# faustomorales/keras-ocr

Hardware: AMD Instinct MI355X
Metric: images/sec end-to-end Pipeline.recognize() @768x768 (higher is better)
Workload: dtype f32 (fp32 operands as 2 fp16 pieces [F(4,3) / head layers] or 3 bf16 pieces [1x1, dilated], 3 / 6 MFMA products, fp32 accumulate; fp32-class error vs fp64: tests/test_conv_gpu.py)

## Files before the change

### keras_ocr_amd/csrc/conv_w43h.hip

```cpp
#include "w43_common.h"
#include "probe_clock.h"

namespace {

#define W4H_SCALED_CONSTANTS(sc)                                                                       \
  const float k_s = (sc), k_sA = (sc) * W4_A, k_sB = (sc) * W4_B, k_sA2 = (sc) * W4_A2, k_sB2 = (sc) * W4_B2, \
              k_sA2B2 = (sc) * W4_A2B2, k_sA2PB2 = (sc) * W4_A2PB2
template <class T>
__device__ __forceinline__ T w4h_transform(const T (&d)[6], int xi, float k_s, float k_sA, float k_sB, float k_sA2, float k_sB2,
                                           float k_sA2B2, float k_sA2PB2) {
  switch (xi) {
    case 0: return (k_sA2B2 * d[0] - k_sA2PB2 * d[2]) + k_s * d[4];
    case 1: return (k_s * d[4] - k_sB2 * d[2]) + k_sA * (d[3] - W4_B2 * d[1]);
    case 2: return (k_s * d[4] - k_sB2 * d[2]) - k_sA * (d[3] - W4_B2 * d[1]);
    case 3: return (k_s * d[4] - k_sA2 * d[2]) + k_sB * (d[3] - W4_A2 * d[1]);
    case 4: return (k_s * d[4] - k_sA2 * d[2]) - k_sB * (d[3] - W4_A2 * d[1]);
    default: return (k_sA2B2 * d[1] - k_sA2PB2 * d[3]) + k_s * d[5];
  }
}

constexpr int W4H_TOP = 12;

}

template <int POOL, int GEO, int NP, int DBG = 0, int MODE = 0>
__global__ __launch_bounds__(256) void conv_w43vh_kernel(W4Params p) {
  static_assert(GEO == 1 || GEO == 2, "4 x 64 or 8 x 32 tiles");
  static_assert(!(POOL && GEO == 2), "no fused pooling on 8 x 32 tiles");
  static_assert(NP == 1 || NP == 2, "one or two fp16 pieces");
  static_assert(MODE == 0 || MODE == 1 || MODE == 2, "exact tiling, ragged, cells");
  constexpr int PR = NP == 2 ? 3 : 1;
  constexpr int NROWS = GEO == 2 ? 10 : 6;
  constexpr int QPR = GEO == 2 ? 8 : 16;
  constexpr int KHS = QPR * 8;
  constexpr int ROW_STRIDE = 2 * KHS;
  constexpr int PLANE_R = NROWS * 2 * KHS;
  constexpr int BUF_R = 6 * NP * PLANE_R;
  constexpr int TCOLS = QPR * 4;
  extern __shared__ __attribute__((aligned(16))) unsigned short As[];
  float* coef = reinterpret_cast<float*>(As + 2 * BUF_R);
  const int tid = threadIdx.x, lane = tid & 63;
  const int wn = __builtin_amdgcn_readfirstlane(tid >> 6);
  const int l31 = lane & 31, l5 = lane >> 5;
  const int nblk_n = p.Cout_pad >> 7;
  const int total = p.total_tiles;
  const int ncg = p.Cin >> 4;
  const int ns = 3 * ncg;
  const int G = gridDim.x;
  constexpr unsigned OOB = 0x80000000u;
  PROBE_T0();

  auto slot = [&](int w, int kh, int q) {
    if constexpr (GEO == 2)
      return ((w >> 1) * 2 + kh) * 128 + (w & 1) * 64 + ((q * 8) ^ (kh * 32));
    else
      return w * ROW_STRIDE + kh * KHS + ((q * 8) ^ (kh * 32));
  };
  auto tile_org = [&](int mp, int& y0, int& x0, int& nimg_o) -> long {
    if constexpr (MODE != 0) {
      const int rq = (int)w4_fdiv((unsigned)mp, p.dv_tpr), cb = mp - rq * p.tiles_per_row;
      const int nimg = (int)w4_fdiv((unsigned)rq, p.dv_rq), ro = rq - nimg * p.rq_per_img;
      y0 = (GEO == 2 ? 8 : 4) * ro;
      x0 = TCOLS * cb;
      nimg_o = nimg;
      return ((long)nimg * p.H + y0) * p.W + x0;
    } else if constexpr (GEO == 2) {
      const int rq = (int)w4_fdiv((unsigned)mp, p.dv_tpr), cb = mp - rq * p.tiles_per_row;
      const int ho = p.H >> 3;
      const int nimg = (int)w4_fdiv((unsigned)rq, p.dv_hh), ro = rq - nimg * ho;
      y0 = 8 * ro;
      x0 = 32 * cb;
      return ((long)nimg * p.H + y0) * p.W + x0;
    } else {
      const int rq = (int)w4_fdiv((unsigned)mp, p.dv_tpr), cb = mp - rq * p.tiles_per_row;
      return w4_mtile_pm0<1>(p, 2 * rq * p.tiles_per_row + cb, y0, x0);
    }
  };

  const int q4 = tid & 3, qd0 = (tid >> 2) & (QPR - 1), r0 = GEO == 2 ? (tid >> 5) : (tid >> 6);
  const int cp = tid & 7;
  const int qd1 = GEO == 2 ? ((tid >> 3) & 7) : ((tid >> 3) & 15);
  const int r1 = GEO == 2 ? 8 + ((tid >> 6) & 1) : 4 + (tid >> 7);
  int ldst[2];
  ldst[0] = slot(r0, q4 >> 1, qd0) + (q4 & 1) * 4;
  ldst[1] = slot(r1, cp >> 2, qd1) + (cp & 3) * 2;
  struct Geo {
    unsigned off0[2];
    unsigned ok;
    int e;
    int e1, qb;
    const float* base;
  };
  auto make_geo = [&](int L, Geo& g, bool& left, bool& right) __attribute__((always_inline)) {
    int mp, nt_unused;
    w4_decode(p, kocr_xcd_remap(L < total ? L : 0, total), nblk_n, mp, nt_unused);
    int y0, x0, nimg = 0;
    const long pm = tile_org(mp, y0, x0, nimg);
    g.base = p.in + (pm * p.in_cs + p.in_co) - (long)(p.W + 1) * p.in_cs;
    const int tid = wn * 64 + kocr_fresh_lane();
    const int q4 = tid & 3, qd0 = (tid >> 2) & (QPR - 1), r0 = GEO == 2 ? (tid >> 5) : (tid >> 6);
    const int cp = tid & 7;
    const int qd1 = GEO == 2 ? ((tid >> 3) & 7) : ((tid >> 3) & 15);
    const int r1 = GEO == 2 ? 8 + ((tid >> 6) & 1) : 4 + (tid >> 7);
    g.off0[0] = (unsigned)(((r0 * p.W + 4 * qd0) * p.in_cs + q4 * 4) * 4);
    g.off0[1] = (unsigned)(((r1 * p.W + 4 * qd1) * p.in_cs + cp * 2) * 4);
    g.ok = ((L < total && (unsigned)(y0 - 1 + r0) < (unsigned)p.H) ? 1u : 0u) |
           ((L < total && (unsigned)(y0 - 1 + r1) < (unsigned)p.H) ? 2u : 0u);
    g.e1 = 0;
    g.qb = QPR;
    if constexpr (MODE == 2) {
      const int j0 = (int)w4_fdiv((unsigned)x0, p.dv_wc);
      const int j1 = j0 + 1 < p.cells_per_row ? j0 + 1 : j0;
      const int c0 = __builtin_amdgcn_readfirstlane(nimg * p.cells_per_row + j0), c1 = __builtin_amdgcn_readfirstlane(nimg * p.cells_per_row + j1);
      g.e = kocr_scale_exp_bits(kocr_sload(p.amax_in + c0), W4H_TOP);
      g.e1 = kocr_scale_exp_bits(kocr_sload(p.amax_in + c1), W4H_TOP);
      const int qb = ((j0 + 1) * p.cellW - x0) >> 2;
      g.qb = qb < QPR ? qb : QPR;
    } else if constexpr (MODE == 1) {
      g.e = kocr_scale_exp_bits(kocr_sload(p.amax_in + __builtin_amdgcn_readfirstlane(nimg)), W4H_TOP);
    } else {
      g.e = kocr_scale_exp_bits(kocr_sload(p.amax_in + __builtin_amdgcn_readfirstlane((int)w4_fdiv((unsigned)pm, p.dv_hw))), W4H_TOP);
    }
    if constexpr (MODE == 1) {
      const int c0 = x0 - 1 + 4 * qd0, c1 = x0 - 1 + 4 * qd1;
      unsigned cm = 0;
#pragma unroll
      for (int k = 0; k < 6; ++k)
        cm |= ((unsigned)(c0 + k) < (unsigned)p.W ? 0u : (4u << k)) | ((unsigned)(c1 + k) < (unsigned)p.W ? 0u : (256u << k));
      g.ok |= cm;
      left = right = false;
    } else {
      left = x0 == 0;
      right = x0 + TCOLS >= p.W;
    }
  };
  Geo gc, gn;
  bool lc, rc, ln, rn;
  int ld_cg = 0;
  bool ld_next = false;
  auto load_item0 = [&](v4f (&raw)[6]) __attribute__((always_inline)) {
    if constexpr (DBG & 16) return;
    const int soff = ld_cg * 64;
    const unsigned okb = ld_next ? gn.ok : gc.ok;
    const bool ok = okb & 1u;
    const unsigned off0 = (ld_next ? gn.off0[0] : gc.off0[0]) | (ok ? 0u : OOB);
    const bool left = (ld_next ? ln : lc) && qd0 == 0, right = (ld_next ? rn : rc) && qd0 == QPR - 1;
    const unsigned stride = (unsigned)(p.in_cs * 4);
    const __amdgpu_buffer_rsrc_t rsrc = w4_rsrc(ld_next ? gn.base : gc.base, 0x80000000u);
#pragma unroll
    for (int k = 0; k < 6; ++k) {
      const unsigned padk = MODE == 1 ? ((okb << (29 - k)) & OOB)
                                      : ((k == 0 ? (left ? OOB : 0u) : 0u) | (k == 5 ? (right ? OOB : 0u) : 0u));
      if constexpr (DBG & 128)
        raw[k] = __builtin_bit_cast(v4f, __builtin_amdgcn_raw_buffer_load_b128(w4_rsrc(p.in, 0x80000000u), (unsigned)((tid & 63) * 16 + (tid >> 6) * 8192 + k * 1024), soff & 0xFFF, 0));
      else if constexpr (DBG & 64)
        raw[k] = __builtin_bit_cast(v4f, __builtin_amdgcn_raw_buffer_load_b128(w4_rsrc(p.in, 0x80000000u), ((off0 + k * stride) | padk) & 0x8003FFF0u, soff & 0xFFF, 0));
      else
      raw[k] = __builtin_bit_cast(v4f, __builtin_amdgcn_raw_buffer_load_b128(rsrc, (off0 + k * stride) | padk, soff, 0));
    }
  };
  auto load_item1 = [&](v2f (&raw)[6]) __attribute__((always_inline)) {
    if constexpr (DBG & 16) return;
    const int soff = ld_cg * 64;
    const unsigned okb = ld_next ? gn.ok : gc.ok;
    const bool ok = (okb >> 1) & 1u;
    const unsigned off0 = (ld_next ? gn.off0[1] : gc.off0[1]) | (ok ? 0u : OOB);
    const bool left = (ld_next ? ln : lc) && qd1 == 0, right = (ld_next ? rn : rc) && qd1 == QPR - 1;
    const unsigned stride = (unsigned)(p.in_cs * 4);
    const __amdgpu_buffer_rsrc_t rsrc = w4_rsrc(ld_next ? gn.base : gc.base, 0x80000000u);
#pragma unroll
    for (int k = 0; k < 6; ++k) {
      const unsigned padk = MODE == 1 ? ((okb << (23 - k)) & OOB)
                                      : ((k == 0 ? (left ? OOB : 0u) : 0u) | (k == 5 ? (right ? OOB : 0u) : 0u));
      if constexpr (DBG & 128)
        raw[k] = __builtin_bit_cast(v2f, __builtin_amdgcn_raw_buffer_load_b64(w4_rsrc(p.in, 0x80000000u), (unsigned)((tid & 63) * 8 + (tid >> 6) * 8192 + 6144 + k * 512), soff & 0xFFF, 0));
      else if constexpr (DBG & 64)
        raw[k] = __builtin_bit_cast(v2f, __builtin_amdgcn_raw_buffer_load_b64(w4_rsrc(p.in, 0x80000000u), ((off0 + k * stride) | padk) & 0x8003FFF8u, soff & 0xFFF, 0));
      else
      raw[k] = __builtin_bit_cast(v2f, __builtin_amdgcn_raw_buffer_load_b64(rsrc, (off0 + k * stride) | padk, soff, 0));
    }
  };
  auto advance = [&]() __attribute__((always_inline)) {
    const bool wrap = ld_cg == ncg - 1;
    ld_cg = wrap ? 0 : ld_cg + 1;
    ld_next = ld_next || wrap;
  };
  auto produce4 = [&](const v4f (&d)[6], unsigned short* bufp, int xi, int it, float sc0, float sc1, int scq) __attribute__((always_inline)) {
    const float sk = MODE == 2 ? (qd0 < scq ? sc0 : sc1) : sc0;
    unsigned short* dst = bufp + xi * NP * PLANE_R + ldst[it];
    if constexpr (DBG & 1) {
      const u2v r = __builtin_bit_cast(u2v, __builtin_shufflevector(d[xi], d[xi], 0, 1));
      *reinterpret_cast<u2v*>(dst) = r;
      if constexpr (NP == 2) *reinterpret_cast<u2v*>(dst + PLANE_R) = r;
      return;
    }
    v4f V;
    if constexpr (MODE == 2) {
      V = w4_transform(d, xi) * sk;
    } else {
      W4H_SCALED_CONSTANTS(sk);
      V = w4h_transform(d, xi, k_s, k_sA, k_sB, k_sA2, k_sB2, k_sA2B2, k_sA2PB2);
    }
    if constexpr (NP == 2) {
      u2v h, l;
      kocr_split4_h(V, h, l);
      *reinterpret_cast<u2v*>(dst) = h;
      *reinterpret_cast<u2v*>(dst + PLANE_R) = l;
    } else {
      *reinterpret_cast<u2v*>(dst) = u2v{__builtin_bit_cast(unsigned, hf2{(_Float16)V[0], (_Float16)V[1]}),
                                         __builtin_bit_cast(unsigned, hf2{(_Float16)V[2], (_Float16)V[3]})};
    }
  };
  auto produce2 = [&](const v2f (&d)[6], unsigned short* bufp, int xi, float sc0, float sc1, int scq) __attribute__((always_inline)) {
    const float sk = MODE == 2 ? (qd1 < scq ? sc0 : sc1) : sc0;
    unsigned short* dst = bufp + xi * NP * PLANE_R + ldst[1];
    if constexpr (DBG & 1) {
      const unsigned r = __float_as_uint(d[xi][0]);
      *reinterpret_cast<unsigned*>(dst) = r;
      if constexpr (NP == 2) *reinterpret_cast<unsigned*>(dst + PLANE_R) = r;
      return;
    }
    v2f V;
    if constexpr (MODE == 2) {
      V = w4_transform(d, xi) * sk;
    } else {
      W4H_SCALED_CONSTANTS(sk);
      V = w4h_transform(d, xi, k_s, k_sA, k_sB, k_sA2, k_sB2, k_sA2B2, k_sA2PB2);
    }
    if constexpr (NP == 2) {
      unsigned h, l;
      kocr_split2_h(V, h, l);
      *reinterpret_cast<unsigned*>(dst) = h;
      *reinterpret_cast<unsigned*>(dst + PLANE_R) = l;
    } else {
      *reinterpret_cast<unsigned*>(dst) = __builtin_bit_cast(unsigned, hf2{(_Float16)V[0], (_Float16)V[1]});
    }
  };
  v4f raw0[6];
  v2f raw1[6];

  const int ntiles32 = p.Cout_pad >> 5;
  const unsigned w_step = (unsigned)ntiles32 * 12 * 64 * 16;
  const __amdgpu_buffer_rsrc_t wrsrc = w4_rsrc(reinterpret_cast<const float*>(p.wgt), 0x7FFFFFFFu);
  const unsigned wlane = (unsigned)lane * 16u;
  auto w_tile = [&](int nt) { return (unsigned)__builtin_amdgcn_readfirstlane((nt * 4 + wn) * 12 * 64 * 16); };
  hf8 bw[2][6][NP];
  f16v acc[6][2];
  const int a_lane = GEO == 2 ? slot(l31 >> 3, l5, l31 & 7) : slot(l31 >> 4, l5, l31 & 15);
  const int a_lane1 = GEO == 2 ? slot((l31 >> 3) + 1, l5, l31 & 7) : 0;
  auto load_a = [&](hf8 (&a)[2][NP], const unsigned short* bufp, int ky, int xi) __attribute__((always_inline)) {
    if constexpr (DBG & 8) return;
    const unsigned short* plane = bufp + xi * NP * PLANE_R;
#pragma unroll
    for (int s = NP - 1; s >= 0; --s)
#pragma unroll
      for (int m = 0; m < 2; ++m) {
        int off;
        if constexpr (GEO == 2) {
          const int c = ky + 4 * m;
          off = ((c & 1) ? a_lane1 : a_lane) + (c >> 1) * 256;
        } else {
          off = a_lane + (ky + 2 * m) * ROW_STRIDE;
        }
        a[m][s] = *reinterpret_cast<const hf8*>(plane + s * PLANE_R + off);
      }
  };
  auto mfma_pt = [&](const hf8 (&a)[2][NP], const hf8 (&b)[NP], int xi) __attribute__((always_inline)) {
    if constexpr (DBG & 4) {
#pragma unroll
      for (int m = 0; m < 2; ++m)
#pragma unroll
        for (int s = 0; s < NP; ++s) acc[xi][m][s] += __builtin_bit_cast(v4f, a[m][s])[0] + __builtin_bit_cast(v4f, b[s])[0];
      return;
    }
    if constexpr (NP == 2) {
#pragma unroll
      for (int m = 0; m < 2; ++m) acc[xi][m] = __builtin_amdgcn_mfma_f32_32x32x16_f16(a[m][1], b[0], acc[xi][m], 0, 0, 0);
#pragma unroll
      for (int m = 0; m < 2; ++m) acc[xi][m] = __builtin_amdgcn_mfma_f32_32x32x16_f16(a[m][0], b[1], acc[xi][m], 0, 0, 0);
    }
#pragma unroll
    for (int m = 0; m < 2; ++m) acc[xi][m] = __builtin_amdgcn_mfma_f32_32x32x16_f16(a[m][0], b[0], acc[xi][m], 0, 0, 0);
  };
  hf8 a0[2][NP], a1[2][NP];
  auto step = [&](auto ky_c, auto slot_c, const unsigned short* bufc, unsigned short* bufn, unsigned w_next, float sc0, float sc1, int scq) __attribute__((always_inline)) {
    constexpr int KY = decltype(ky_c)::value;
    constexpr int SLOT = decltype(slot_c)::value;
    auto load_b = [&](int xi) __attribute__((always_inline)) {
      if constexpr (DBG & 2) return;
#pragma unroll
      for (int s = 0; s < NP; ++s)
        bw[SLOT][xi][s] = __builtin_bit_cast(hf8, __builtin_amdgcn_raw_buffer_load_b128(wrsrc, wlane, (int)(w_next + (unsigned)(xi * 2 + s) * 1024u), 0));
    };
    auto produce = [&](int xi) __attribute__((always_inline)) {
      if constexpr (KY == 0) produce4(raw0, bufn, xi, 0, sc0, sc1, scq);
      if constexpr (KY == 1) produce2(raw1, bufn, xi, sc0, sc1, scq);
    };
    auto interleave = [&]() __attribute__((always_inline)) {
      __builtin_amdgcn_sched_group_barrier(0x100, 2 * NP, 0);
      if constexpr (KY < 2) {
        constexpr int VPG = (KY == 0 ? 30 : 16) / (2 * PR - 1) + 1;
#pragma unroll
        for (int i = 0; i < 2 * PR - 1; ++i) {
          __builtin_amdgcn_sched_group_barrier(0x008, 1, 0);
          __builtin_amdgcn_sched_group_barrier(0x002, VPG, 0);
        }
        __builtin_amdgcn_sched_group_barrier(0x200, NP, 0);
        __builtin_amdgcn_sched_group_barrier(0x008, 1, 0);
      } else {
        __builtin_amdgcn_sched_group_barrier(0x008, 2 * PR, 0);
      }
    };
#pragma unroll
    for (int q = 0; q < 3; ++q) {
      __builtin_amdgcn_sched_barrier(0);
      load_a(a1, bufc, KY, 2 * q + 1);
      produce(2 * q);
      mfma_pt(a0, bw[SLOT][2 * q], 2 * q);
      interleave();
      __builtin_amdgcn_sched_barrier(0);
      load_b(2 * q);
      __builtin_amdgcn_sched_barrier(0);
      if (q < 2) {
        load_a(a0, bufc, KY, 2 * q + 2);
        produce(2 * q + 1);
        mfma_pt(a1, bw[SLOT][2 * q + 1], 2 * q + 1);
        interleave();
      } else if constexpr (KY < 2) {
        load_a(a0, bufc, KY + 1, 0);
        produce(5);
        mfma_pt(a1, bw[SLOT][5], 5);
        interleave();
      } else {
        if constexpr (!(DBG & 32)) __syncthreads();
        load_a(a0, bufn, 0, 0);
        __builtin_amdgcn_sched_barrier(0);
        mfma_pt(a1, bw[SLOT][5], 5);
      }
      __builtin_amdgcn_sched_barrier(0);
      load_b(2 * q + 1);
    }
  };

  w4_stage_coef(p, coef, tid);
  make_geo(blockIdx.x, gc, lc, rc);
  make_geo(blockIdx.x + G, gn, ln, rn);
  load_item0(raw0);
  load_item1(raw1);
  advance();
  {
    int mp0, nt0;
    w4_decode(p, kocr_xcd_remap(blockIdx.x, total), nblk_n, mp0, nt0);
    const unsigned w0 = w_tile(nt0);
#pragma unroll
    for (int st = 0; st < 2; ++st)
#pragma unroll
      for (int xi = 0; xi < 6; ++xi)
#pragma unroll
        for (int s = 0; s < NP; ++s)
          bw[st][xi][s] = __builtin_bit_cast(hf8, __builtin_amdgcn_raw_buffer_load_b128(wrsrc, wlane, (int)(w0 + st * w_step + (unsigned)(xi * 2 + s) * 1024u), 0));
  }
#pragma unroll
  for (int xi = 0; xi < 6; ++xi) {
    produce4(raw0, As, xi, 0, kocr_pow2(gc.e), kocr_pow2(gc.e1), gc.qb);
    produce2(raw1, As, xi, kocr_pow2(gc.e), kocr_pow2(gc.e1), gc.qb);
  }
  load_item0(raw0);
  load_item1(raw1);
  advance();
  __syncthreads();
  load_a(a0, As, 0, 0);

  PROBE_RESTART();
  for (int L = blockIdx.x; L < total; L += G) {
    int mp, nt, mp_n, nt_n;
    w4_decode(p, kocr_xcd_remap(L, total), nblk_n, mp, nt);
    w4_decode(p, kocr_xcd_remap(L + G < total ? L + G : L, total), nblk_n, mp_n, nt_n);
    const unsigned w_ptr = w_tile(nt), w_after = w_tile(nt_n);
    auto w_at = [&](int s) { return s < ns ? w_ptr + (unsigned)s * w_step : w_after + (unsigned)(s - ns) * w_step; };
    const float s_cur = kocr_pow2(gc.e), s_nxt = kocr_pow2(gn.e);
    const float s_cur1 = kocr_pow2(gc.e1), s_nxt1 = kocr_pow2(gn.e1);
    const int qb_nxt = gn.qb;
    const float unscale = kocr_pow2(-gc.e);
    const float unscale1 = kocr_pow2(-gc.e1);
    const int qb_cur = gc.qb;
#pragma unroll
    for (int x = 0; x < 6; ++x)
#pragma unroll
      for (int m = 0; m < 2; ++m)
#pragma unroll
        for (int r = 0; r < 16; ++r) acc[x][m][r] = 0.f;
    PROBE_T(5);
    __builtin_amdgcn_s_waitcnt(0x0F70);
    PROBE_T(4);
    for (int cg = 0; cg < ncg; cg += 2) {
      using I0 = std::integral_constant<int, 0>;
      using I1 = std::integral_constant<int, 1>;
      using I2 = std::integral_constant<int, 2>;
      step(I0{}, I0{}, As, As + BUF_R, w_at(3 * cg + 2), s_cur, s_cur1, qb_cur);
      load_item0(raw0);
      step(I1{}, I1{}, As, As + BUF_R, w_at(3 * cg + 3), s_cur, s_cur1, qb_cur);
      load_item1(raw1);
      advance();
      step(I2{}, I0{}, As, As + BUF_R, w_at(3 * cg + 4), s_cur, s_cur1, qb_cur);
      const bool same = cg + 2 < ncg;
      const float s_odd = same ? s_cur : s_nxt, s_odd1 = same ? s_cur1 : s_nxt1;
      const int qb_odd = same ? qb_cur : qb_nxt;
      step(I0{}, I1{}, As + BUF_R, As, w_at(3 * cg + 5), s_odd, s_odd1, qb_odd);
      load_item0(raw0);
      step(I1{}, I0{}, As + BUF_R, As, w_at(3 * cg + 6), s_odd, s_odd1, qb_odd);
      load_item1(raw1);
      advance();
      step(I2{}, I1{}, As + BUF_R, As, w_at(3 * cg + 7), s_odd, s_odd1, qb_odd);
    }
    PROBE_T(0);

    {
      const int lane_e = kocr_fresh_lane();
      const int l31e = lane_e & 31, l5e = lane_e >> 5;
      const int n = (nt * 4 + wn) * 32 + l31e;
      int ty0, tx0, timg = 0;
      const long tpm = tile_org(mp, ty0, tx0, timg);
      int nimg, nimg1 = 0, cell0_x = 0;
      if constexpr (MODE == 2) {
        const int j0 = (int)w4_fdiv((unsigned)tx0, p.dv_wc);
        const int j1 = j0 + 1 < p.cells_per_row ? j0 + 1 : j0;
        nimg = __builtin_amdgcn_readfirstlane(timg * p.cells_per_row + j0);
        nimg1 = __builtin_amdgcn_readfirstlane(timg * p.cells_per_row + j1);
        cell0_x = j0 * p.cellW;
      } else if constexpr (MODE == 1) {
        nimg = __builtin_amdgcn_readfirstlane(timg);
      } else {
        nimg = __builtin_amdgcn_readfirstlane((int)w4_fdiv((unsigned)tpm, p.dv_hw));
      }
      const unsigned seen_out = p.amax_out ? kocr_amax_peek(p.amax_out + nimg) : 0u;
      const unsigned seen_pool = p.amax_pool ? kocr_amax_peek(p.amax_pool + nimg) : 0u;
      unsigned seen_out1 = 0u, seen_pool1 = 0u;
      if constexpr (MODE == 2) {
        seen_out1 = p.amax_out ? kocr_amax_peek(p.amax_out + nimg1) : 0u;
        seen_pool1 = p.amax_pool ? kocr_amax_peek(p.amax_pool + nimg1) : 0u;
      }
      const float pa = coef[n] * unscale, pb = coef[p.Cout_pad + n];
      const float pa1 = coef[n] * unscale1;
      const bool has_post = p.post_a != nullptr;
      const float qa = coef[2 * p.Cout_pad + n], qb = coef[3 * p.Cout_pad + n];
      const bool live = n < p.Cout;
      const float lo = p.relu ? 0.f : -INFINITY;
      auto act = [&](float v, float a) { return fmaxf(v * a + pb, lo); };
      const int l5q = 4 * l5e;
      auto qx_of = [&](int r) { return GEO == 2 ? (r & 3) + l5q : (r & 3) + 8 * ((r >> 2) & 1) + l5q; };
      auto first_row = [&](int m, int r) { return m == 0 && (GEO == 2 ? (r >> 2) == 0 : r < 8); };
#pragma unroll
      for (int m = 0; m < 2; ++m)
#pragma unroll
        for (int r = 0; r < 16; ++r) {
          float par = pa;
          if constexpr (MODE == 2) par = qx_of(r) < qb_cur ? pa : pa1;
          const float m0 = acc[0][m][r], m1 = acc[1][m][r], m2 = acc[2][m][r], m3 = acc[3][m][r], m4 = acc[4][m][r],
                      m5 = acc[5][m][r];
          const float s12 = m1 + m2, d12 = m1 - m2, s34 = m3 + m4, d34 = m3 - m4;
          acc[0][m][r] = act((m0 + s12) + s34, par);
          acc[1][m][r] = act(W4_A * d12 + W4_B * d34, par);
          acc[2][m][r] = act(W4_A2 * s12 + W4_B2 * s34, par);
          acc[3][m][r] = act((W4_A3 * d12 + W4_B3 * d34) + m5, par);
        }
      if (has_post) {
#pragma unroll
        for (int j = 0; j < 4; ++j)
#pragma unroll
          for (int m = 0; m < 2; ++m)
#pragma unroll
            for (int r = 0; r < 16; ++r) acc[j][m][r] = acc[j][m][r] * qa + qb;
      }
      if constexpr (MODE == 2) {
        const bool top = ty0 == 0;
#pragma unroll
        for (int r = 0; r < 16; ++r) {
          const int qx = qx_of(r);
          const int cx = tx0 + 4 * qx - (qx < qb_cur ? cell0_x : cell0_x + p.cellW);
#pragma unroll
          for (int j = 0; j < 4; ++j) {
            const bool v = cx + j < p.cellWv;
#pragma unroll
            for (int m = 0; m < 2; ++m) acc[j][m][r] = (v && !(top && first_row(m, r))) ? acc[j][m][r] : 0.f;
          }
        }
      }
      int ocs4 = p.out_cs * 4;
      asm volatile("" : "+s"(ocs4));
      int pcs4 = p.pool_cs * 4;
      asm volatile("" : "+s"(pcs4));
      if (p.amax_out || p.amax_pool) {
        if constexpr (MODE == 2) {
          float mx0 = 0.f, mx1 = 0.f;
#pragma unroll
          for (int r = 0; r < 16; ++r) {
            float mq = 0.f;
#pragma unroll
            for (int j = 0; j < 4; ++j)
#pragma unroll
              for (int m = 0; m < 2; ++m) mq = fmaxf(mq, fabsf(acc[j][m][r]));
            const bool first = qx_of(r) < qb_cur;
            mx0 = fmaxf(mx0, first ? mq : 0.f);
            mx1 = fmaxf(mx1, first ? 0.f : mq);
          }
          mx0 = live ? mx0 : 0.f;
          mx1 = live ? mx1 : 0.f;
          if (p.amax_out) kocr_amax_update_known(p.amax_out + nimg, mx0, seen_out);
          if (p.amax_pool) kocr_amax_update_known(p.amax_pool + nimg, mx0, seen_pool);
          if (qb_cur < QPR) {
            if (p.amax_out) kocr_amax_update_known(p.amax_out + nimg1, mx1, seen_out1);
            if (p.amax_pool) kocr_amax_update_known(p.amax_pool + nimg1, mx1, seen_pool1);
          }
        } else {
          float mx = 0.f;
#pragma unroll
          for (int j = 0; j < 4; ++j)
#pragma unroll
            for (int m = 0; m < 2; ++m)
#pragma unroll
              for (int r = 0; r < 16; ++r) mx = fmaxf(mx, fabsf(acc[j][m][r]));
          mx = live ? mx : 0.f;
          if (p.amax_out) kocr_amax_update_known(p.amax_out + nimg, mx, seen_out);
          if (p.amax_pool) kocr_amax_update_known(p.amax_pool + nimg, mx, seen_pool);
        }
      }
      PROBE_T(2);
      if constexpr (GEO == 2) {
        const __amdgpu_buffer_rsrc_t ro = w4_rsrc(p.out + (tpm * p.out_cs + p.out_co), 0x7FFFFFFFu);
        const unsigned vo = live ? (unsigned)((16 * l5e * p.out_cs + n) * 4) : OOB;
        const int wlim = p.W - tx0 - 16 * l5e;
#pragma unroll
        for (int m = 0; m < 2; ++m)
#pragma unroll
          for (int r = 0; r < 16; ++r) {
            const int px = (4 * m + (r >> 2)) * p.W + 4 * (r & 3);
            if (MODE == 1 && ty0 + 4 * m + (r >> 2) >= p.H) continue;
#pragma unroll
            for (int j = 0; j < 4; ++j) {
              const unsigned vom = MODE == 1 ? (4 * (r & 3) + j < wlim ? vo : OOB) : vo;
              __builtin_amdgcn_raw_buffer_store_b32(__float_as_uint(acc[j][m][r]), ro, vom, (px + j) * ocs4, 0);
            }
          }
      } else {
#pragma unroll
        for (int m = 0; m < 2; ++m) {
          const long pm = tpm + (long)2 * m * p.W;
          const int x0 = tx0;
          if (!POOL || p.write_full) {
            const __amdgpu_buffer_rsrc_t ro = w4_rsrc(p.out + (pm * p.out_cs + p.out_co), 0x7FFFFFFFu);
            const unsigned vo = live ? (unsigned)((16 * l5e * p.out_cs + n) * 4) : OOB;
            if constexpr (MODE == 1) {
              const int wlim = p.W - tx0 - 16 * l5e;
#pragma unroll
              for (int h = 0; h < 2; ++h) {
                if (ty0 + 2 * m + h >= p.H) continue;
#pragma unroll
                for (int r = 0; r < 8; ++r) {
                  const int px = 4 * ((r & 3) + 8 * (r >> 2));
#pragma unroll
                  for (int j = 0; j < 4; ++j)
                    __builtin_amdgcn_raw_buffer_store_b32(__float_as_uint(acc[j][m][r + 8 * h]), ro, px + j < wlim ? vo : OOB,
                                                          (px + j + h * p.W) * ocs4, 0);
                }
              }
            } else {
#pragma unroll
              for (int r = 0; r < 8; ++r) {
                const int px = 4 * ((r & 3) + 8 * (r >> 2));
#pragma unroll
                for (int j = 0; j < 4; ++j) {
                  __builtin_amdgcn_raw_buffer_store_b32(__float_as_uint(acc[j][m][r]), ro, vo, (px + j) * ocs4, 0);
                  __builtin_amdgcn_raw_buffer_store_b32(__float_as_uint(acc[j][m][r + 8]), ro, vo, (px + j + p.W) * ocs4, 0);
                }
              }
            }
          }
          if constexpr (POOL) {
            long pp0;
            if constexpr (MODE == 1)
              pp0 = ((long)timg * (p.H >> 1) + (ty0 >> 1) + m) * (p.W >> 1) + (x0 >> 1);
            else
              pp0 = ((pm - x0) >> 2) + (x0 >> 1);
            const __amdgpu_buffer_rsrc_t rp = w4_rsrc(p.pool_out + (pp0 * p.pool_cs + p.pool_co), 0x7FFFFFFFu);
            const unsigned vp = live ? (unsigned)((8 * l5e * p.pool_cs + n) * 4) : OOB;
            if (MODE == 1 && (ty0 >> 1) + m >= (p.H >> 1)) continue;
            const int plim = (p.W >> 1) - (x0 >> 1) - 8 * l5e;
            const bool ztop = MODE == 2 && ty0 == 0 && m == 0;
#pragma unroll
            for (int r = 0; r < 8; ++r) {
              const int pq = 2 * ((r & 3) + 8 * (r >> 2));
              float v0 = fmaxf(fmaxf(acc[0][m][r], acc[1][m][r]), fmaxf(acc[0][m][r + 8], acc[1][m][r + 8]));
              float v1 = fmaxf(fmaxf(acc[2][m][r], acc[3][m][r]), fmaxf(acc[2][m][r + 8], acc[3][m][r + 8]));
              if constexpr (MODE == 2) {
                v0 = ztop ? 0.f : v0;
                v1 = ztop ? 0.f : v1;
              }
              __builtin_amdgcn_raw_buffer_store_b32(__float_as_uint(v0), rp, (MODE != 1 || pq < plim) ? vp : OOB, pq * pcs4, 0);
              __builtin_amdgcn_raw_buffer_store_b32(__float_as_uint(v1), rp, (MODE != 1 || pq + 1 < plim) ? vp : OOB, (pq + 1) * pcs4, 0);
            }
          }
        }
      }
      PROBE_T(3);
    }
    gc = gn;
    lc = ln;
    rc = rn;
    make_geo(L + 2 * G, gn, ln, rn);
    ld_next = false;
    PROBE_T(1);
  }
  PROBE_TEND(tid == 0, 0, 6);
}

template <int POOL, int NP, int MODE = 0, int OCC = 1>
__global__ __launch_bounds__(256, OCC) void conv_w43rh_kernel(W4Params p) {
  static_assert(MODE == 0 || MODE == 1, "exact tiling or ragged");
  constexpr int NBW = 3;
  constexpr int PR = NP == 2 ? 3 : 1;
  constexpr int NROWS = 6, QPR = 16, KHS = QPR * 8, ROW_STRIDE = 2 * KHS, PLANE_R = NROWS * ROW_STRIDE;
  constexpr int BUF_R = 6 * NP * PLANE_R;
  constexpr int TCOLS = QPR * 4;
  extern __shared__ __attribute__((aligned(16))) unsigned short As[];
  float* coef = reinterpret_cast<float*>(OCC == 2 ? As + 2 * BUF_R : As + BUF_R + 4 * 16 * 64 * 8);
  const int tid = threadIdx.x, lane = tid & 63;
  const int wave = __builtin_amdgcn_readfirstlane(tid >> 6);
  const int wn = wave & 1, ph = wave >> 1;
  const int l31 = lane & 31, l5 = lane >> 5;
  const int total = p.total_tiles;
  const int ncg = p.Cin >> 4;
  const int G = gridDim.x;
  constexpr unsigned OOB = 0x80000000u;

  auto tile_mt = [&](int mp, int m) {
    const int rq = (int)w4_fdiv((unsigned)mp, p.dv_tpr), cb = mp - rq * p.tiles_per_row;
    return (2 * rq + m) * p.tiles_per_row + cb;
  };
  auto mtile_org = [&](int mp, int m, int& y0, int& x0, int& nimg_o) -> long {
    if constexpr (MODE == 1) {
      const int rq = (int)w4_fdiv((unsigned)mp, p.dv_tpr), cb = mp - rq * p.tiles_per_row;
      const int nimg = (int)w4_fdiv((unsigned)rq, p.dv_rq), ro = rq - nimg * p.rq_per_img;
      y0 = 4 * ro + 2 * m;
      x0 = TCOLS * cb;
      nimg_o = nimg;
      return ((long)nimg * p.H + y0) * p.W + x0;
    } else {
      const long pm = w4_mtile_pm0<1>(p, tile_mt(mp, m), y0, x0);
      nimg_o = (int)w4_fdiv((unsigned)pm, p.dv_hw);
      return pm;
    }
  };

  const int q4 = tid & 3, qd0 = (tid >> 2) & (QPR - 1), r0 = tid >> 6;
  const int cp = tid & 7, qd1 = (tid >> 3) & 15, r1 = 4 + (tid >> 7);
  int ldst[2];
  ldst[0] = r0 * ROW_STRIDE + (q4 >> 1) * KHS + (((qd0 * 8) ^ ((q4 >> 1) * 32)) + (q4 & 1) * 4);
  ldst[1] = r1 * ROW_STRIDE + (cp >> 2) * KHS + (((qd1 * 8) ^ ((cp >> 2) * 32)) + (cp & 3) * 2);
  struct Geo {
    unsigned off0[2];
    unsigned ok;
    int e;
    const float* base;
  };
  auto make_geo = [&](int L, Geo& g, bool& left, bool& right) __attribute__((always_inline)) {
    const int mp = kocr_xcd_remap(L < total ? L : 0, total);
    int y0, x0, nimg;
    const long pm = mtile_org(mp, 0, y0, x0, nimg);
    g.base = p.in + (pm * p.in_cs + p.in_co) - (long)(p.W + 1) * p.in_cs;
    const int tid = wave * 64 + kocr_fresh_lane();
    const int q4 = tid & 3, qd0 = (tid >> 2) & (QPR - 1), r0 = tid >> 6;
    const int cp = tid & 7, qd1 = (tid >> 3) & 15, r1 = 4 + (tid >> 7);
    g.off0[0] = (unsigned)(((r0 * p.W + 4 * qd0) * p.in_cs + q4 * 4) * 4);
    g.off0[1] = (unsigned)(((r1 * p.W + 4 * qd1) * p.in_cs + cp * 2) * 4);
    g.ok = ((L < total && (unsigned)(y0 - 1 + r0) < (unsigned)p.H) ? 1u : 0u) |
           ((L < total && (unsigned)(y0 - 1 + r1) < (unsigned)p.H) ? 2u : 0u);
    g.e = kocr_scale_exp_bits(kocr_sload(p.amax_in + __builtin_amdgcn_readfirstlane(nimg)), W4H_TOP);
    if constexpr (MODE == 1) {
      const int c0 = x0 - 1 + 4 * qd0, c1 = x0 - 1 + 4 * qd1;
      unsigned cm = 0;
#pragma unroll
      for (int k = 0; k < 6; ++k)
        cm |= ((unsigned)(c0 + k) < (unsigned)p.W ? 0u : (4u << k)) | ((unsigned)(c1 + k) < (unsigned)p.W ? 0u : (256u << k));
      g.ok |= cm;
      left = right = false;
    } else {
      left = x0 == 0;
      right = x0 + TCOLS >= p.W;
    }
  };
  Geo gc, gn;
  bool lc, rc, ln, rn;
  int ld_cg = 0;
  bool ld_next = false;
  auto load_item0 = [&](v4f (&raw)[6]) __attribute__((always_inline)) {
    const int soff = ld_cg * 64;
    const unsigned okb = ld_next ? gn.ok : gc.ok;
    const bool ok = okb & 1u;
    const unsigned off0 = (ld_next ? gn.off0[0] : gc.off0[0]) | (ok ? 0u : OOB);
    const bool left = (ld_next ? ln : lc) && qd0 == 0, right = (ld_next ? rn : rc) && qd0 == QPR - 1;
    const unsigned stride = (unsigned)(p.in_cs * 4);
    const __amdgpu_buffer_rsrc_t rsrc = w4_rsrc(ld_next ? gn.base : gc.base, 0x80000000u);
#pragma unroll
    for (int k = 0; k < 6; ++k) {
      const unsigned padk = MODE == 1 ? ((okb << (29 - k)) & OOB) : ((k == 0 ? (left ? OOB : 0u) : 0u) | (k == 5 ? (right ? OOB : 0u) : 0u));
      raw[k] = __builtin_bit_cast(v4f, __builtin_amdgcn_raw_buffer_load_b128(rsrc, (off0 + k * stride) | padk, soff, 0));
    }
  };
  auto load_item1 = [&](v2f (&raw)[6]) __attribute__((always_inline)) {
    const int soff = ld_cg * 64;
    const unsigned okb = ld_next ? gn.ok : gc.ok;
    const bool ok = (okb >> 1) & 1u;
    const unsigned off0 = (ld_next ? gn.off0[1] : gc.off0[1]) | (ok ? 0u : OOB);
    const bool left = (ld_next ? ln : lc) && qd1 == 0, right = (ld_next ? rn : rc) && qd1 == QPR - 1;
    const unsigned stride = (unsigned)(p.in_cs * 4);
    const __amdgpu_buffer_rsrc_t rsrc = w4_rsrc(ld_next ? gn.base : gc.base, 0x80000000u);
#pragma unroll
    for (int k = 0; k < 6; ++k) {
      const unsigned padk = MODE == 1 ? ((okb << (23 - k)) & OOB) : ((k == 0 ? (left ? OOB : 0u) : 0u) | (k == 5 ? (right ? OOB : 0u) : 0u));
      raw[k] = __builtin_bit_cast(v2f, __builtin_amdgcn_raw_buffer_load_b64(rsrc, (off0 + k * stride) | padk, soff, 0));
    }
  };
  auto advance = [&]() __attribute__((always_inline)) {
    const bool wrap = ld_cg == ncg - 1;
    ld_cg = wrap ? 0 : ld_cg + 1;
    ld_next = ld_next || wrap;
  };
  auto produce4 = [&](const v4f (&d)[6], unsigned short* bufp, int xi, float sk) __attribute__((always_inline)) {
    W4H_SCALED_CONSTANTS(sk);
    const v4f V = w4h_transform(d, xi, k_s, k_sA, k_sB, k_sA2, k_sB2, k_sA2B2, k_sA2PB2);
    unsigned short* dst = bufp + xi * NP * PLANE_R + ldst[0];
    if constexpr (NP == 2) {
      u2v h, l;
      kocr_split4_h(V, h, l);
      *reinterpret_cast<u2v*>(dst) = h;
      *reinterpret_cast<u2v*>(dst + PLANE_R) = l;
    } else {
      *reinterpret_cast<u2v*>(dst) = u2v{__builtin_bit_cast(unsigned, hf2{(_Float16)V[0], (_Float16)V[1]}),
                                         __builtin_bit_cast(unsigned, hf2{(_Float16)V[2], (_Float16)V[3]})};
    }
  };
  auto produce2 = [&](const v2f (&d)[6], unsigned short* bufp, int xi, float sk) __attribute__((always_inline)) {
    W4H_SCALED_CONSTANTS(sk);
    const v2f V = w4h_transform(d, xi, k_s, k_sA, k_sB, k_sA2, k_sB2, k_sA2B2, k_sA2PB2);
    unsigned short* dst = bufp + xi * NP * PLANE_R + ldst[1];
    if constexpr (NP == 2) {
      unsigned h, l;
      kocr_split2_h(V, h, l);
      *reinterpret_cast<unsigned*>(dst) = h;
      *reinterpret_cast<unsigned*>(dst + PLANE_R) = l;
    } else {
      *reinterpret_cast<unsigned*>(dst) = __builtin_bit_cast(unsigned, hf2{(_Float16)V[0], (_Float16)V[1]});
    }
  };
  v4f raw0[1][6];
  v2f raw1[1][6];

  constexpr unsigned w_step = 2u * 12 * 64 * 16;
  const __amdgpu_buffer_rsrc_t wrsrc = w4_rsrc(reinterpret_cast<const float*>(p.wgt), 0x7FFFFFFFu);
  const unsigned wlane = (unsigned)lane * 16u;
  const unsigned w_wave = (unsigned)__builtin_amdgcn_readfirstlane(wn * 12 * 64 * 16 + 3 * ph * 2 * 64 * 16);
  const int ns = 3 * ncg;
  hf8 bw[NBW][NP];
  f16v acc[3][2];
  const int a_lane = (l31 >> 4) * ROW_STRIDE + l5 * KHS + (((l31 & 15) * 8) ^ (l5 * 32));
  constexpr int M_OFF = 2 * ROW_STRIDE;
  auto load_a = [&](hf8 (&a)[2][NP], const unsigned short* bufp, int ky, int pl) __attribute__((always_inline)) {
    const unsigned short* base = bufp + a_lane + ky * ROW_STRIDE + (3 * ph + pl) * NP * PLANE_R;
#pragma unroll
    for (int s = NP - 1; s >= 0; --s)
#pragma unroll
      for (int m = 0; m < 2; ++m) a[m][s] = *reinterpret_cast<const hf8*>(base + s * PLANE_R + m * M_OFF);
  };
  auto mfma_grp = [&](const hf8 (&a)[2][NP], int pl, int bi) __attribute__((always_inline)) {
    if constexpr (NP == 2) {
#pragma unroll
      for (int m = 0; m < 2; ++m) acc[pl][m] = __builtin_amdgcn_mfma_f32_32x32x16_f16(a[m][1], bw[bi][0], acc[pl][m], 0, 0, 0);
#pragma unroll
      for (int m = 0; m < 2; ++m) acc[pl][m] = __builtin_amdgcn_mfma_f32_32x32x16_f16(a[m][0], bw[bi][1], acc[pl][m], 0, 0, 0);
    }
#pragma unroll
    for (int m = 0; m < 2; ++m) acc[pl][m] = __builtin_amdgcn_mfma_f32_32x32x16_f16(a[m][0], bw[bi][0], acc[pl][m], 0, 0, 0);
  };
  hf8 a0[2][NP], a1[2][NP];
  auto phase = [&](const unsigned short* bufc, unsigned short* bufn, int s0, int flip, float sk) __attribute__((always_inline)) {
    v4f(&r0)[6] = raw0[0];
    v2f(&r1)[6] = raw1[0];
#pragma unroll
    for (int g = 0; g < 9; ++g) {
      __builtin_amdgcn_sched_barrier(0);
      const int ky = g / 3, pp = g - ky * 3;
      hf8(&cur)[2][NP] = ((g & 1) ^ flip) ? a1 : a0;
      hf8(&nxt)[2][NP] = ((g & 1) ^ flip) ? a0 : a1;
      const int nchunks = (g % 3 == 0) ? 2 : 1;
      const int c0 = (g / 3) * 4 + (g % 3 == 0 ? 0 : g % 3 + 1);
      if (g < 8) load_a(nxt, bufc, (g + 1) / 3, (g + 1) % 3);
#pragma unroll
      for (int c = c0; c < c0 + nchunks; ++c) {
        if (c < 6)
          produce4(r0, bufn, c, sk);
        else
          produce2(r1, bufn, c - 6, sk);
      }
      if (g < 8) {
        mfma_grp(cur, pp, pp);
        __builtin_amdgcn_sched_group_barrier(0x100, 2 * NP, 0);
        auto ilv = [&](auto v_c, auto st_c) __attribute__((always_inline)) {
          constexpr int V = decltype(v_c)::value, ST = decltype(st_c)::value;
#pragma unroll
          for (int i = 0; i < 2 * PR - 1; ++i) {
            __builtin_amdgcn_sched_group_barrier(0x008, 1, 0);
            __builtin_amdgcn_sched_group_barrier(0x002, V, 0);
          }
          __builtin_amdgcn_sched_group_barrier(0x200, ST, 0);
        };
        const bool half = c0 >= 6;
        if (nchunks == 2) {
          if (half)
            ilv(std::integral_constant<int, PR == 3 ? 3 : 20>{}, std::integral_constant<int, 2 * NP>{});
          else
            ilv(std::integral_constant<int, PR == 3 ? 5 : 44>{}, std::integral_constant<int, 2 * NP>{});
        } else {
          if (half)
            ilv(std::integral_constant<int, PR == 3 ? 2 : 10>{}, std::integral_constant<int, NP>{});
          else
            ilv(std::integral_constant<int, PR == 3 ? 2 : 22>{}, std::integral_constant<int, NP>{});
        }
        __builtin_amdgcn_sched_group_barrier(0x008, 1, 0);
      } else {
        __syncthreads();
        load_a(nxt, bufn, 0, 0);
        __builtin_amdgcn_sched_barrier(0);
        mfma_grp(cur, pp, pp);
      }
      __builtin_amdgcn_sched_barrier(0);
      {
        int sn = s0 + ky + 1;
        sn = sn >= ns ? sn - ns : sn;
        const unsigned wq = w_wave + (unsigned)sn * w_step;
#pragma unroll
        for (int s = 0; s < NP; ++s)
          bw[pp][s] = __builtin_bit_cast(hf8, __builtin_amdgcn_raw_buffer_load_b128(wrsrc, wlane, (int)(wq + (unsigned)(pp * 2 + s) * 1024u), 0));
      }
      if (g == 3) load_item0(r0);
    }
    load_item1(r1);
    advance();
  };

  w4_stage_coef(p, coef, tid);
  make_geo(blockIdx.x, gc, lc, rc);
  make_geo(blockIdx.x + G, gn, ln, rn);
  load_item0(raw0[0]);
  load_item1(raw1[0]);
  advance();
#pragma unroll
  for (int g = 0; g < NBW; ++g)
#pragma unroll
    for (int s = 0; s < NP; ++s)
      bw[g][s] = __builtin_bit_cast(hf8, __builtin_amdgcn_raw_buffer_load_b128(wrsrc, wlane, (int)(w_wave + (unsigned)(g / 3) * w_step + (unsigned)((g % 3) * 2 + s) * 1024u), 0));
#pragma unroll
  for (int xi = 0; xi < 6; ++xi) {
    produce4(raw0[0], As, xi, kocr_pow2(gc.e));
    produce2(raw1[0], As, xi, kocr_pow2(gc.e));
  }
  load_item0(raw0[0]);
  load_item1(raw1[0]);
  advance();
  __syncthreads();
  load_a(a0, As, 0, 0);

  PROBE_T0();
  for (int L = blockIdx.x; L < total; L += G) {
    const int mp = kocr_xcd_remap(L, total);
    const float s_cur = kocr_pow2(gc.e), s_nxt = kocr_pow2(gn.e);
    const float unscale = kocr_pow2(-gc.e);
#pragma unroll
    for (int x = 0; x < 3; ++x)
#pragma unroll
      for (int m = 0; m < 2; ++m)
#pragma unroll
        for (int r = 0; r < 16; ++r) acc[x][m][r] = 0.f;
    PROBE_T(5);
    __builtin_amdgcn_s_waitcnt(0x0F70);
    PROBE_T(4);
    for (int cg = 0; cg < ncg; cg += 2) {
      phase(As, As + BUF_R, 3 * cg, 0, s_cur);
      phase(As + BUF_R, As, 3 * cg + 3, 1, cg + 2 < ncg ? s_cur : s_nxt);
    }

    PROBE_T(0);
    {
      const int lane_e = kocr_fresh_lane();
      const int l31e = lane_e & 31, l5e = lane_e >> 5;
      const int n = wn * 32 + l31e;
      int y0, x0, timg;
      const long pm = mtile_org(mp, ph, y0, x0, timg);
      const int nimg = __builtin_amdgcn_readfirstlane(timg);
      const unsigned seen_out = p.amax_out ? kocr_amax_peek(p.amax_out + nimg) : 0u;
      const unsigned seen_pool = p.amax_pool ? kocr_amax_peek(p.amax_pool + nimg) : 0u;
      const float pa = coef[n] * unscale, pb = coef[p.Cout_pad + n];
      const bool has_post = p.post_a != nullptr;
      const float qa = coef[2 * p.Cout_pad + n], qb = coef[3 * p.Cout_pad + n];
      const bool live = n < p.Cout;
      const float lo = p.relu ? 0.f : -INFINITY;
      auto act = [&](float v) { return fmaxf(v * pa + pb, lo); };
      v4f* xch = reinterpret_cast<v4f*>(As + BUF_R);
      float out[4][16];
      auto halves = [&](auto ph_c) __attribute__((always_inline)) {
        constexpr int PH = decltype(ph_c)::value;
        auto partial = [&](auto m_c, int r, float (&o)[4]) __attribute__((always_inline)) {
          constexpr int M = decltype(m_c)::value;
          const float u = acc[0][M][r], v = acc[1][M][r], w = acc[2][M][r];
          if constexpr (PH == 0) {
            const float s12 = v + w, d12 = v - w;
            o[0] = u + s12;
            o[1] = W4_A * d12;
            o[2] = W4_A2 * s12;
            o[3] = W4_A3 * d12;
          } else {
            const float s34 = u + v, d34 = u - v;
            o[0] = s34;
            o[1] = W4_B * d34;
            o[2] = W4_B2 * s34;
            o[3] = W4_B3 * d34 + w;
          }
        };
        if constexpr (OCC == 1) {
#pragma unroll
          for (int r = 0; r < 16; ++r) {
            float o[4];
            partial(std::integral_constant<int, 1 - PH>{}, r, o);
            xch[(wave * 16 + r) * 64 + lane_e] = v4f{o[0], o[1], o[2], o[3]};
          }
        }
#pragma unroll
        for (int r = 0; r < 16; ++r) {
          float o[4];
          partial(std::integral_constant<int, PH>{}, r, o);
#pragma unroll
          for (int j = 0; j < 4; ++j) out[j][r] = o[j];
        }
        if constexpr (OCC == 2) {
#pragma unroll
          for (int h = 0; h < 2; ++h) {
#pragma unroll
            for (int r = 8 * h; r < 8 * h + 8; ++r) {
              float o[4];
              partial(std::integral_constant<int, 1 - PH>{}, r, o);
              xch[(wave * 8 + r - 8 * h) * 64 + lane_e] = v4f{o[0], o[1], o[2], o[3]};
            }
            __syncthreads();
#pragma unroll
            for (int r = 8 * h; r < 8 * h + 8; ++r) {
              const v4f q = xch[((wave ^ 2) * 8 + r - 8 * h) * 64 + lane_e];
#pragma unroll
              for (int j = 0; j < 4; ++j) out[j][r] += q[j];
            }
            __syncthreads();
          }
        }
      };
      if (ph == 0)
        halves(std::integral_constant<int, 0>{});
      else
        halves(std::integral_constant<int, 1>{});
      if constexpr (OCC == 1) {
        __syncthreads();
#pragma unroll
        for (int r = 0; r < 16; ++r) {
          const v4f q = xch[((wave ^ 2) * 16 + r) * 64 + lane_e];
#pragma unroll
          for (int j = 0; j < 4; ++j) out[j][r] = act(out[j][r] + q[j]);
        }
      } else {
#pragma unroll
        for (int r = 0; r < 16; ++r)
#pragma unroll
          for (int j = 0; j < 4; ++j) out[j][r] = act(out[j][r]);
      }
      if (has_post) {
#pragma unroll
        for (int r = 0; r < 16; ++r)
#pragma unroll
          for (int j = 0; j < 4; ++j) out[j][r] = out[j][r] * qa + qb;
      }
      if constexpr (OCC == 1) __syncthreads();
      int ocs4 = p.out_cs * 4;
      asm volatile("" : "+s"(ocs4));
      int pcs4 = p.pool_cs * 4;
      asm volatile("" : "+s"(pcs4));
      if (p.amax_out || p.amax_pool) {
        float mx = 0.f;
#pragma unroll
        for (int j = 0; j < 4; ++j)
#pragma unroll
          for (int r = 0; r < 16; ++r) mx = fmaxf(mx, fabsf(out[j][r]));
        mx = live ? mx : 0.f;
        if (p.amax_out) kocr_amax_update_known(p.amax_out + nimg, mx, seen_out);
        if (p.amax_pool) kocr_amax_update_known(p.amax_pool + nimg, mx, seen_pool);
      }
      PROBE_T(2);
      if (!POOL || p.write_full) {
        const __amdgpu_buffer_rsrc_t ro = w4_rsrc(p.out + (pm * p.out_cs + p.out_co), 0x7FFFFFFFu);
        const unsigned vo = live ? (unsigned)((16 * l5e * p.out_cs + n) * 4) : OOB;
        if constexpr (MODE == 1) {
          const int wlim = p.W - x0 - 16 * l5e;
#pragma unroll
          for (int h = 0; h < 2; ++h) {
            if (y0 + h >= p.H) continue;
#pragma unroll
            for (int r = 0; r < 8; ++r) {
              const int px = 4 * ((r & 3) + 8 * (r >> 2));
#pragma unroll
              for (int j = 0; j < 4; ++j)
                __builtin_amdgcn_raw_buffer_store_b32(__float_as_uint(out[j][r + 8 * h]), ro, px + j < wlim ? vo : OOB, (px + j + h * p.W) * ocs4, 0);
            }
          }
        } else {
#pragma unroll
          for (int r = 0; r < 8; ++r) {
            const int px = 4 * ((r & 3) + 8 * (r >> 2));
#pragma unroll
            for (int j = 0; j < 4; ++j) {
              __builtin_amdgcn_raw_buffer_store_b32(__float_as_uint(out[j][r]), ro, vo, (px + j) * ocs4, 0);
              __builtin_amdgcn_raw_buffer_store_b32(__float_as_uint(out[j][r + 8]), ro, vo, (px + j + p.W) * ocs4, 0);
            }
          }
        }
      }
      if constexpr (POOL) {
        long pp0;
        if constexpr (MODE == 1)
          pp0 = ((long)timg * (p.H >> 1) + (y0 >> 1)) * (p.W >> 1) + (x0 >> 1);
        else
          pp0 = ((pm - x0) >> 2) + (x0 >> 1);
        const __amdgpu_buffer_rsrc_t rp = w4_rsrc(p.pool_out + (pp0 * p.pool_cs + p.pool_co), 0x7FFFFFFFu);
        const unsigned vp = live ? (unsigned)((8 * l5e * p.pool_cs + n) * 4) : OOB;
        const bool prow = MODE != 1 || (y0 >> 1) < (p.H >> 1);
        const int plim = (p.W >> 1) - (x0 >> 1) - 8 * l5e;
        if (prow) {
#pragma unroll
          for (int r = 0; r < 8; ++r) {
            const int pq = 2 * ((r & 3) + 8 * (r >> 2));
            const float v0 = fmaxf(fmaxf(out[0][r], out[1][r]), fmaxf(out[0][r + 8], out[1][r + 8]));
            const float v1 = fmaxf(fmaxf(out[2][r], out[3][r]), fmaxf(out[2][r + 8], out[3][r + 8]));
            __builtin_amdgcn_raw_buffer_store_b32(__float_as_uint(v0), rp, (MODE != 1 || pq < plim) ? vp : OOB, pq * pcs4, 0);
            __builtin_amdgcn_raw_buffer_store_b32(__float_as_uint(v1), rp, (MODE != 1 || pq + 1 < plim) ? vp : OOB, (pq + 1) * pcs4, 0);
          }
        }
      }
      PROBE_T(3);
    }
    gc = gn;
    lc = ln;
    rc = rn;
    make_geo(L + 2 * G, gn, ln, rn);
    ld_next = false;
    PROBE_T(1);
  }
  PROBE_TEND(tid == 0, 0, 6);
}

template <int NP, int DIL = 0>
__global__ __launch_bounds__(256) void conv_w43fh_kernel(W4Params p) {
  constexpr int PR = NP == 2 ? 3 : 1;
  constexpr int PLANE_F = PLANE;
  constexpr int BUF_F = 6 * NP * PLANE_F;
  extern __shared__ __attribute__((aligned(16))) unsigned short As[];
  float* coef = reinterpret_cast<float*>(As + 2 * BUF_F);
  const int tid = threadIdx.x, lane = tid & 63;
  const int wn = __builtin_amdgcn_readfirstlane(tid >> 6);
  const int l31 = lane & 31, l5 = lane >> 5;
  const int nblk_n = p.Cout_pad >> 7;
  const int total = p.total_tiles;
  const int ns = p.nsteps;
  const int G = gridDim.x;
  const int hw = p.H * p.W;
  constexpr unsigned OOB = 0x80000000u;

  const int qi = tid >> 2, q4 = tid & 3;
  const int ldst = ((qi >> 5) * 2 + (q4 >> 1)) * KH_STRIDE + ((((qi & 31) * 8) ^ ((q4 >> 1) * 32)) + (q4 & 1) * 4);
  struct Geo {
    unsigned goff[6];
    int gy;
    bool gok;
    float s;
    int e0, e1;
    const float* base;
  };
  const int dd = DIL ? p.dil : 1;
  auto make_geo = [&](int L, Geo& g) __attribute__((always_inline)) {
    int mp, nt_unused;
    w4_decode(p, kocr_xcd_remap(L < total ? L : 0, total), nblk_n, mp, nt_unused);
    const int tid_f = wn * 64 + kocr_fresh_lane();
    const int qi = tid_f >> 2, q4 = tid_f & 3;
    if constexpr (DIL) {
      const unsigned q0 = (unsigned)mp * 64u;
      const unsigned nq = (unsigned)(p.Mtotal >> 2);
      const unsigned row_a = w4_fdiv(q0 < nq ? q0 : nq - 1, p.dv_qpr);
      g.base = p.in + ((long)row_a * p.W * p.in_cs + p.in_co) - (long)(dd * p.W + dd) * p.in_cs;
      const unsigned qg = q0 + (unsigned)qi;
      g.gok = L < total && qg < nq;
      const unsigned qc = qg < nq ? qg : nq - 1;
      const unsigned row = w4_fdiv(qc, p.dv_qpr);
      const int qr = (int)(qc - row * (unsigned)p.qpr);
      const int qd = (int)w4_fdiv((unsigned)qr, p.dv_dil);
      const int x0 = qd * 4 * dd + (qr - qd * dd);
      const unsigned nimg = w4_fdiv(row, p.dv_h);
      g.gy = (int)(row - nimg * (unsigned)p.H);
      const int n0 = __builtin_amdgcn_readfirstlane((int)w4_fdiv(row_a, p.dv_h));
      const int n1 = (n0 + 1 < p.Mtotal / (p.H * p.W)) ? n0 + 1 : n0;
      g.e0 = kocr_scale_exp_bits(kocr_sload(p.amax_in + n0), W4H_TOP);
      g.e1 = kocr_scale_exp_bits(kocr_sload(p.amax_in + n1), W4H_TOP);
      g.s = kocr_pow2((int)nimg == n0 ? g.e0 : g.e1);
      const int rel = (int)(row - row_a) * p.W + x0;
#pragma unroll
      for (int k = 0; k < 6; ++k) {
        const bool pad = (k == 0 && x0 < dd) || (k == 5 && x0 + 4 * dd >= p.W);
        g.goff[k] = pad ? OOB : (unsigned)(((rel + k * dd) * p.in_cs + q4 * 4) * 4);
      }
      return;
    }
    const long pm_a = (long)mp * 256;
    g.base = p.in + (pm_a * p.in_cs + p.in_co) - (long)(p.W + 1) * p.in_cs;
    const int rel = 4 * qi;
    const long gp = pm_a + rel;
    g.gok = L < total && gp < p.Mtotal;
    const unsigned gpc = (unsigned)(gp < p.Mtotal ? gp : (long)p.Mtotal - 1);
    const unsigned row = w4_fdiv(gpc, p.dv_w), nimg = w4_fdiv(gpc, p.dv_hw);
    const int x0 = (int)(gpc - row * (unsigned)p.W);
    g.gy = (int)(row - nimg * (unsigned)p.H);
    const unsigned pmc = (unsigned)(pm_a < (long)p.Mtotal ? pm_a : (long)p.Mtotal - 1);
    const int n0 = __builtin_amdgcn_readfirstlane((int)w4_fdiv(pmc, p.dv_hw));
    const int n1 = ((long)(n0 + 1) * hw < (long)p.Mtotal) ? n0 + 1 : n0;
    g.e0 = kocr_scale_exp_bits(kocr_sload(p.amax_in + n0), W4H_TOP);
    g.e1 = kocr_scale_exp_bits(kocr_sload(p.amax_in + n1), W4H_TOP);
    g.s = kocr_pow2((int)nimg == n0 ? g.e0 : g.e1);
#pragma unroll
    for (int k = 0; k < 6; ++k) {
      const bool pad = (k == 0 && x0 < 1) || (k == 5 && x0 + 4 >= p.W);
      g.goff[k] = pad ? OOB : (unsigned)(((rel + k) * p.in_cs + q4 * 4) * 4);
    }
  };
  Geo gc, gn;
  int ld_ky = 0, ld_cg = 0;
  bool ld_next = false;
  const int ncg = p.Cin >> 4;
  auto load_raw = [&](v4f (&raw)[6]) __attribute__((always_inline)) {
    const int soff = (ld_ky * dd * p.W * p.in_cs + ld_cg * 16) * 4;
    const int gy = ld_next ? gn.gy : gc.gy;
    const bool ok = (ld_next ? gn.gok : gc.gok) & ((unsigned)(gy + dd * (ld_ky - 1)) < (unsigned)p.H);
    const unsigned kill = ok ? 0u : OOB;
    const __amdgpu_buffer_rsrc_t rsrc = w4_rsrc(ld_next ? gn.base : gc.base, 0x80000000u);
#pragma unroll
    for (int k = 0; k < 6; ++k)
      raw[k] = __builtin_bit_cast(v4f, __builtin_amdgcn_raw_buffer_load_b128(rsrc, (ld_next ? gn.goff[k] : gc.goff[k]) | kill, soff, 0));
    const bool wrap_ky = ld_ky == 2;
    ld_ky = wrap_ky ? 0 : ld_ky + 1;
    const bool wrap_cg = wrap_ky && ld_cg == ncg - 1;
    ld_cg = wrap_cg ? 0 : (wrap_ky ? ld_cg + 1 : ld_cg);
    ld_next = ld_next || wrap_cg;
  };
  auto produce_point = [&](const v4f (&d)[6], unsigned short* bufp, int xi, float sk) __attribute__((always_inline)) {
    W4H_SCALED_CONSTANTS(sk);
    const v4f V = w4h_transform(d, xi, k_s, k_sA, k_sB, k_sA2, k_sB2, k_sA2B2, k_sA2PB2);
    unsigned short* dst = bufp + xi * NP * PLANE_F + ldst;
    if constexpr (NP == 2) {
      u2v h, l;
      kocr_split4_h(V, h, l);
      *reinterpret_cast<u2v*>(dst) = h;
      *reinterpret_cast<u2v*>(dst + PLANE_F) = l;
    } else {
      *reinterpret_cast<u2v*>(dst) = u2v{__builtin_bit_cast(unsigned, hf2{(_Float16)V[0], (_Float16)V[1]}),
                                         __builtin_bit_cast(unsigned, hf2{(_Float16)V[2], (_Float16)V[3]})};
    }
  };

  const int ntiles32 = p.Cout_pad >> 5;
  const size_t w_step = (size_t)ntiles32 * 12 * 64 * 8;
  auto w_tile = [&](int nt) { return p.wgt + ((size_t)(nt * 4 + wn) * 12 * 64 + lane) * 8; };
  hf8 bw[6][NP];
  f16v acc[6][2];
  const int a_lane = l5 * KH_STRIDE + ((l31 * 8) ^ (l5 * 32));
  auto load_a = [&](hf8 (&a)[2][NP], const unsigned short* bufp, int xi) __attribute__((always_inline)) {
    const unsigned short* base = bufp + xi * NP * PLANE_F + a_lane;
#pragma unroll
    for (int s = NP - 1; s >= 0; --s)
#pragma unroll
      for (int m = 0; m < 2; ++m) a[m][s] = *reinterpret_cast<const hf8*>(base + s * PLANE_F + m * 2 * KH_STRIDE);
  };
  auto mfma_pt = [&](const hf8 (&a)[2][NP], int xi) __attribute__((always_inline)) {
    if constexpr (NP == 2) {
#pragma unroll
      for (int m = 0; m < 2; ++m) acc[xi][m] = __builtin_amdgcn_mfma_f32_32x32x16_f16(a[m][1], bw[xi][0], acc[xi][m], 0, 0, 0);
#pragma unroll
      for (int m = 0; m < 2; ++m) acc[xi][m] = __builtin_amdgcn_mfma_f32_32x32x16_f16(a[m][0], bw[xi][1], acc[xi][m], 0, 0, 0);
    }
#pragma unroll
    for (int m = 0; m < 2; ++m) acc[xi][m] = __builtin_amdgcn_mfma_f32_32x32x16_f16(a[m][0], bw[xi][0], acc[xi][m], 0, 0, 0);
  };
  hf8 a0[2][NP], a1[2][NP];
  auto step = [&](const unsigned short* bufc, unsigned short* bufn, const v4f (&raw)[6], const unsigned short* w_next, float sk)
                  __attribute__((always_inline)) {
    auto load_b = [&](int xi) __attribute__((always_inline)) {
#pragma unroll
      for (int s = 0; s < NP; ++s) bw[xi][s] = *reinterpret_cast<const hf8*>(w_next + (size_t)(xi * 2 + s) * 64 * 8);
    };
    auto interleave = [&]() __attribute__((always_inline)) {
      __builtin_amdgcn_sched_group_barrier(0x100, 2 * NP, 0);
      constexpr int VPG = 30 / (2 * PR - 1) + 1;
#pragma unroll
      for (int i = 0; i < 2 * PR - 1; ++i) {
        __builtin_amdgcn_sched_group_barrier(0x008, 1, 0);
        __builtin_amdgcn_sched_group_barrier(0x002, VPG, 0);
      }
      __builtin_amdgcn_sched_group_barrier(0x200, NP, 0);
      __builtin_amdgcn_sched_group_barrier(0x008, 1, 0);
    };
#pragma unroll
    for (int q = 0; q < 3; ++q) {
      __builtin_amdgcn_sched_barrier(0);
      load_a(a1, bufc, 2 * q + 1);
      produce_point(raw, bufn, 2 * q, sk);
      mfma_pt(a0, 2 * q);
      interleave();
      __builtin_amdgcn_sched_barrier(0);
      load_b(2 * q);
      __builtin_amdgcn_sched_barrier(0);
      if (q < 2) {
        load_a(a0, bufc, 2 * q + 2);
        produce_point(raw, bufn, 2 * q + 1, sk);
        mfma_pt(a1, 2 * q + 1);
        interleave();
      } else {
        produce_point(raw, bufn, 5, sk);
        __syncthreads();
        load_a(a0, bufn, 0);
        __builtin_amdgcn_sched_barrier(0);
        mfma_pt(a1, 5);
      }
      __builtin_amdgcn_sched_barrier(0);
      load_b(2 * q + 1);
    }
  };

  w4_stage_coef(p, coef, tid);
  make_geo(blockIdx.x, gc);
  make_geo(blockIdx.x + G, gn);
  v4f rawA[6], rawB[6];
  load_raw(rawA);
  load_raw(rawB);
  {
    int mp0, nt0;
    w4_decode(p, kocr_xcd_remap(blockIdx.x, total), nblk_n, mp0, nt0);
    const unsigned short* w0 = w_tile(nt0);
#pragma unroll
    for (int xi = 0; xi < 6; ++xi)
#pragma unroll
      for (int s = 0; s < NP; ++s) bw[xi][s] = *reinterpret_cast<const hf8*>(w0 + (size_t)(xi * 2 + s) * 64 * 8);
  }
#pragma unroll
  for (int xi = 0; xi < 6; ++xi) produce_point(rawA, As, xi, gc.s);
  load_raw(rawA);
  __syncthreads();
  load_a(a0, As, 0);

  PROBE_T0();
  for (int L = blockIdx.x; L < total; L += G) {
    int mp, nt, mp_n, nt_n;
    w4_decode(p, kocr_xcd_remap(L, total), nblk_n, mp, nt);
    w4_decode(p, kocr_xcd_remap(L + G < total ? L + G : L, total), nblk_n, mp_n, nt_n);
    const unsigned short* w_ptr = w_tile(nt);
    const unsigned short* w_after = w_tile(nt_n);
    const float s_cur = gc.s, s_nxt = gn.s;
#pragma unroll
    for (int x = 0; x < 6; ++x)
#pragma unroll
      for (int m = 0; m < 2; ++m)
#pragma unroll
        for (int r = 0; r < 16; ++r) acc[x][m][r] = 0.f;
    __builtin_amdgcn_s_waitcnt(0x0F70);
    for (int s = 0; s < ns; s += 2) {
      step(As, As + BUF_F, rawB, w_ptr + (size_t)(s + 1) * w_step, s_cur);
      load_raw(rawB);
      step(As + BUF_F, As, rawA, s + 2 < ns ? w_ptr + (size_t)(s + 2) * w_step : w_after, s + 2 < ns ? s_cur : s_nxt);
      load_raw(rawA);
    }
    PROBE_T(0);
    const int e0c = gc.e0, e1c = gc.e1;

    {
      const int lane_e = kocr_fresh_lane();
      const int l31e = lane_e & 31, l5e = lane_e >> 5;
      const int n = (nt * 4 + wn) * 32 + l31e;
      const long pm0 = (long)mp * 256;
      const long pm0c = pm0 < (long)p.Mtotal ? pm0 : (long)p.Mtotal - 1;
      const int n0 = __builtin_amdgcn_readfirstlane((int)w4_fdiv((unsigned)pm0c, p.dv_hw));
      const long b1 = ((long)(n0 + 1) * hw - pm0) >> 2;
      const int qb = __builtin_amdgcn_readfirstlane((int)(b1 < 64 ? b1 : 64));
      const int n1 = ((long)(n0 + 1) * hw < (long)p.Mtotal) ? n0 + 1 : n0;
      unsigned seen0 = 0, seen1 = 0;
      if (p.amax_out) {
        seen0 = kocr_amax_peek(p.amax_out + n0);
        seen1 = kocr_amax_peek(p.amax_out + n1);
      }
      const float u0 = kocr_pow2(-e0c), u1 = kocr_pow2(-e1c);
      const float pre_a = coef[n], pb = coef[p.Cout_pad + n];
      const float pa0 = pre_a * u0, pa1 = pre_a * u1;
      const bool has_post = p.post_a != nullptr;
      const bool live = n < p.Cout;
      const float lo = p.relu ? 0.f : -INFINITY;
      const int qlim = (int)((((long)p.Mtotal - pm0) >> 2) < 64 ? (((long)p.Mtotal - pm0) >> 2) : 64);
      const int l5q = 4 * l5e;
#pragma unroll
      for (int m = 0; m < 2; ++m)
#pragma unroll
        for (int r = 0; r < 16; ++r) {
          const int q = m * 32 + (r & 3) + 8 * (r >> 2) + l5q;
          const float pa = q < qb ? pa0 : pa1;
          const float m0 = acc[0][m][r], m1 = acc[1][m][r], m2 = acc[2][m][r], m3 = acc[3][m][r], m4 = acc[4][m][r],
                      m5 = acc[5][m][r];
          const float s12 = m1 + m2, d12 = m1 - m2, s34 = m3 + m4, d34 = m3 - m4;
          acc[0][m][r] = fmaxf(((m0 + s12) + s34) * pa + pb, lo);
          acc[1][m][r] = fmaxf((W4_A * d12 + W4_B * d34) * pa + pb, lo);
          acc[2][m][r] = fmaxf((W4_A2 * s12 + W4_B2 * s34) * pa + pb, lo);
          acc[3][m][r] = fmaxf(((W4_A3 * d12 + W4_B3 * d34) + m5) * pa + pb, lo);
        }
      if (has_post) {
        const float qa = coef[2 * p.Cout_pad + n], qb_ = coef[3 * p.Cout_pad + n];
#pragma unroll
        for (int j = 0; j < 4; ++j)
#pragma unroll
          for (int m = 0; m < 2; ++m)
#pragma unroll
            for (int r = 0; r < 16; ++r) acc[j][m][r] = acc[j][m][r] * qa + qb_;
      }
      if (!DIL && p.Wv) {
#pragma unroll
        for (int m = 0; m < 2; ++m)
#pragma unroll
          for (int r = 0; r < 16; ++r) {
            const int q = m * 32 + (r & 3) + 8 * (r >> 2) + l5q;
            const unsigned pq = (unsigned)(pm0 + 4 * q);
            const int x0 = (int)(pq - w4_fdiv(pq, p.dv_w) * (unsigned)p.W);
#pragma unroll
            for (int j = 0; j < 4; ++j) acc[j][m][r] = x0 + j < p.Wv ? acc[j][m][r] : 0.f;
          }
      }
      if (p.amax_out) {
        float mx0 = 0.f, mx1 = 0.f;
#pragma unroll
        for (int m = 0; m < 2; ++m)
#pragma unroll
          for (int r = 0; r < 16; ++r) {
            const int q = m * 32 + (r & 3) + 8 * (r >> 2) + l5q;
            const float mq = (live && q < qlim) ? fmaxf(fmaxf(fabsf(acc[0][m][r]), fabsf(acc[1][m][r])), fmaxf(fabsf(acc[2][m][r]), fabsf(acc[3][m][r]))) : 0.f;
            mx0 = fmaxf(mx0, q < qb ? mq : 0.f);
            mx1 = fmaxf(mx1, q < qb ? 0.f : mq);
          }
        kocr_amax_update_known(p.amax_out + n0, mx0, seen0);
        if (qb < 64) kocr_amax_update_known(p.amax_out + n1, mx1, seen1);
      }
      PROBE_T(2);
      int ocs4 = p.out_cs * 4;
      asm volatile("" : "+s"(ocs4));
      if constexpr (DIL) {
        const unsigned q0 = (unsigned)mp * 64u;
        const unsigned row_a = w4_fdiv(q0, p.dv_qpr);
        const __amdgpu_buffer_rsrc_t ro = w4_rsrc(p.out + ((long)row_a * p.W * p.out_cs + p.out_co), 0x7FFFFFFFu);
        const int dstep = dd * ocs4;
#pragma unroll
        for (int m = 0; m < 2; ++m)
#pragma unroll
          for (int r = 0; r < 16; ++r) {
            const int q = m * 32 + (r & 3) + 8 * (r >> 2) + l5q;
            const unsigned qg = q0 + (unsigned)q;
            const unsigned row = w4_fdiv(qg, p.dv_qpr);
            const int qr = (int)(qg - row * (unsigned)p.qpr);
            const int qd = (int)w4_fdiv((unsigned)qr, p.dv_dil);
            const int x0 = qd * 4 * dd + (qr - qd * dd);
            const unsigned vo = (live && q < qlim) ? (unsigned)((((int)(row - row_a) * p.W + x0) * p.out_cs + n) * 4) : OOB;
#pragma unroll
            for (int j = 0; j < 4; ++j) __builtin_amdgcn_raw_buffer_store_b32(__float_as_uint(acc[j][m][r]), ro, vo, j * dstep, 0);
          }
      } else {
      const long rem = ((long)p.Mtotal - pm0) * ocs4;
      const __amdgpu_buffer_rsrc_t ro =
          w4_rsrc(p.out + (pm0 * p.out_cs + p.out_co), rem < 0x7FFFFFFFL ? (unsigned)(rem > 0 ? rem : 0) : 0x7FFFFFFFu);
      const unsigned vo = live ? (unsigned)((16 * l5e * p.out_cs + n) * 4) : OOB;
#pragma unroll
      for (int m = 0; m < 2; ++m)
#pragma unroll
        for (int r = 0; r < 16; ++r) {
          const int px = 4 * (m * 32 + (r & 3) + 8 * (r >> 2));
#pragma unroll
          for (int j = 0; j < 4; ++j)
            __builtin_amdgcn_raw_buffer_store_b32(__float_as_uint(acc[j][m][r]), ro, vo, (px + j) * ocs4, 0);
        }
      }
      PROBE_T(3);
    }
    gc = gn;
    make_geo(L + 2 * G, gn);
    ld_next = false;
    PROBE_T(1);
  }
  PROBE_TEND(tid == 0, 0, 4);
}

int prepare_w43h(kocr_ctx* ctx, ConvLayer& L, const float* w, bool w_is_oihw, const float* pre_a) {
  if (!L.d_w4 || (L.dil != 1 && L.w4_cout_pad == 64)) return KOCR_OK;
  const int Cin = L.Cin, Cout = L.Cout;
  const int cp = L.w4_cout_pad;
  const int nt32 = cp / 32;
  const double pa = W4_PA, pb = W4_PB, a2 = pa * pa, b2 = pb * pb;
  const double na = 2.0 * a2 * (a2 - b2), nb = 2.0 * b2 * (b2 - a2);
  auto U6 = [&](int c, int ky, int o, double (&U)[6]) {
    double g[3];
    for (int kx = 0; kx < 3; ++kx)
      g[kx] = w_is_oihw ? w[(((size_t)o * Cin + c) * 3 + ky) * 3 + kx] : w[(((size_t)ky * 3 + kx) * Cin + c) * Cout + o];
    U[0] = g[0] / (a2 * b2);
    U[1] = (g[0] + pa * g[1] + a2 * g[2]) / na;
    U[2] = (g[0] - pa * g[1] + a2 * g[2]) / na;
    U[3] = (g[0] + pb * g[1] + b2 * g[2]) / nb;
    U[4] = (g[0] - pb * g[1] + b2 * g[2]) / nb;
    U[5] = g[2];
  };
  std::vector<int> wexp(cp, 0);
  for (int o = 0; o < Cout; ++o) {
    double umax = 0;
    for (int c = 0; c < Cin; ++c)
      for (int ky = 0; ky < 3; ++ky) {
        double U[6];
        U6(c, ky, o, U);
        for (int xi = 0; xi < 6; ++xi) umax = std::max(umax, std::fabs(U[xi]));
      }
    if (umax > 0 && std::isfinite(umax)) {
      int E;
      std::frexp((float)umax, &E);
      wexp[o] = std::max(-100, std::min(100, 15 - E));
    }
  }
  std::vector<unsigned short> u((size_t)(Cin / 16) * 3 * nt32 * 12 * 64 * 8, 0);
  for (int c = 0; c < Cin; ++c)
    for (int ky = 0; ky < 3; ++ky)
      for (int o = 0; o < Cout; ++o) {
        double U[6];
        U6(c, ky, o, U);
        const int k = c % 16, lane = (k >> 3) * 32 + (o & 31), j = k & 7;
        const size_t step = (size_t)(c / 16) * 3 + ky;
        for (int xi = 0; xi < 6; ++xi) {
          const float x = std::ldexp((float)U[xi], wexp[o]);
          const _Float16 h = (_Float16)x, l = (_Float16)(x - (float)h);
          unsigned short hb, lb;
          memcpy(&hb, &h, 2);
          memcpy(&lb, &l, 2);
          u[((((step * nt32 + o / 32) * 6 + xi) * 2 + 0) * 64 + lane) * 8 + j] = hb;
          u[((((step * nt32 + o / 32) * 6 + xi) * 2 + 1) * 64 + lane) * 8 + j] = lb;
        }
      }
  void* d = nullptr;
  KOCR_TRY(ctx->dev_alloc(&d, u.size() * sizeof(unsigned short)));
  KOCR_HIP(ctx, hipMemcpy(d, u.data(), u.size() * sizeof(unsigned short), hipMemcpyHostToDevice));
  L.d_w4h = (unsigned short*)d;
  std::vector<float> ah(std::max(cp, L.Cout_pad), 1.f);
  for (int o = 0; o < Cout; ++o) ah[o] = std::ldexp(pre_a ? pre_a[o] : 1.f, -wexp[o]);
  KOCR_TRY(ctx->upload(&L.d_pre_a_h, ah));
  return KOCR_OK;
}

template <int POOL, int GEO, int NP, int DBG = 0, int MODE = 0>
static int w4vh_launch(kocr_ctx* ctx, W4Params& p) {
  constexpr int LDSV0 = (GEO == 2 ? 2 * 6 * 10 * 128 * 2 : 2 * 6 * 6 * 256 * 2) * NP;
  const int LDSV = LDSV0 + 4 * p.Cout_pad * 4;
  int grid;
  PROBE_RESET(ctx);
  KOCR_TRY((launch_persistent<conv_w43vh_kernel<POOL, GEO, NP, DBG, MODE>>(ctx, p, p.total_tiles, 256, LDSV, LDSV0 + W4_COEF_BYTES_MAX,
                                                                           1, &grid)));
  {
    char what[80];
    snprintf(what, sizeof what, "conv_w43vh<%d,%d,%d,%d> tiles %d steps %d cout %d", POOL, GEO, NP, MODE, p.total_tiles, p.nsteps, p.Cout);
    (void)what;
    PROBE_REPORT(ctx, what, grid);
  }
  return KOCR_OK;
}

int launch_w43vh(kocr_ctx* ctx, W4Params& p, bool fuse, int geo, int pieces, int mode) {
  if (mode == 2) {
    if (geo == 2) return w4vh_launch<0, 2, 2, 0, 2>(ctx, p);
    return fuse ? w4vh_launch<1, 1, 2, 0, 2>(ctx, p) : w4vh_launch<0, 1, 2, 0, 2>(ctx, p);
  }
  if (mode == 1) {
    if (geo == 2) return w4vh_launch<0, 2, 2, 0, 1>(ctx, p);
    return fuse ? w4vh_launch<1, 1, 2, 0, 1>(ctx, p) : w4vh_launch<0, 1, 2, 0, 1>(ctx, p);
  }
#ifdef KOCR_DEV_SWITCHES
  static const int dbg = getenv("KOCR_W43H_DBG") ? atoi(getenv("KOCR_W43H_DBG")) : 0;
  if (dbg && !fuse && geo == 1 && pieces == 2) {
    switch (dbg) {
      case 1: return w4vh_launch<0, 1, 2, 1>(ctx, p);
      case 2: return w4vh_launch<0, 1, 2, 2>(ctx, p);
      case 4: return w4vh_launch<0, 1, 2, 4>(ctx, p);
      case 8: return w4vh_launch<0, 1, 2, 8>(ctx, p);
      case 16: return w4vh_launch<0, 1, 2, 16>(ctx, p);
      case 32: return w4vh_launch<0, 1, 2, 32>(ctx, p);
      case 3: return w4vh_launch<0, 1, 2, 3>(ctx, p);
      case 18: return w4vh_launch<0, 1, 2, 18>(ctx, p);
      case 19: return w4vh_launch<0, 1, 2, 19>(ctx, p);
      case 27: return w4vh_launch<0, 1, 2, 27>(ctx, p);
      case 59: return w4vh_launch<0, 1, 2, 59>(ctx, p);
      case 12: return w4vh_launch<0, 1, 2, 12>(ctx, p);
      case 17: return w4vh_launch<0, 1, 2, 17>(ctx, p);
      case 64: return w4vh_launch<0, 1, 2, 64>(ctx, p);
      case 128: return w4vh_launch<0, 1, 2, 128>(ctx, p);
      case 66: return w4vh_launch<0, 1, 2, 66>(ctx, p);
      default: break;
    }
  }
#endif
  if (pieces == 2) {
    if (geo == 2) return w4vh_launch<0, 2, 2>(ctx, p);
    return fuse ? w4vh_launch<1, 1, 2>(ctx, p) : w4vh_launch<0, 1, 2>(ctx, p);
  }
  if (geo == 2) return w4vh_launch<0, 2, 1>(ctx, p);
  return fuse ? w4vh_launch<1, 1, 1>(ctx, p) : w4vh_launch<0, 1, 1>(ctx, p);
}

template <int POOL, int NP, int MODE = 0, int OCC = 1>
static int w4rh_launch(kocr_ctx* ctx, W4Params& p) {
  constexpr int LDSR0 = OCC == 2 ? 2 * 6 * NP * 6 * 256 * 2 : 6 * NP * 6 * 256 * 2 + 4 * 16 * 64 * 16;
  const int LDSR = LDSR0 + 4 * p.Cout_pad * 4;
  int grid;
  PROBE_RESET(ctx);
  KOCR_TRY((launch_persistent<conv_w43rh_kernel<POOL, NP, MODE, OCC>>(ctx, p, p.total_tiles, 256, LDSR, LDSR0 + W4_COEF_BYTES_MAX, OCC,
                                                                       &grid)));
  {
    char what[80];
    snprintf(what, sizeof what, "conv_w43rh<%d,%d,%d,occ%d> tiles %d steps %d", POOL, NP, MODE, OCC, p.total_tiles, p.nsteps);
    (void)what;
    PROBE_REPORT(ctx, what, grid);
  }
  return KOCR_OK;
}

int launch_w43rh(kocr_ctx* ctx, W4Params& p, bool fuse, int pieces, int mode) {
  if (mode == 1) return fuse ? w4rh_launch<1, 2, 1, 2>(ctx, p) : w4rh_launch<0, 2, 1, 2>(ctx, p);
  if (pieces == 2) return fuse ? w4rh_launch<1, 2, 0, 2>(ctx, p) : w4rh_launch<0, 2, 0, 2>(ctx, p);
  return fuse ? w4rh_launch<1, 1>(ctx, p) : w4rh_launch<0, 1>(ctx, p);
}

template <int NP, int DIL = 0>
static int w4fh_launch(kocr_ctx* ctx, W4Params& p) {
  constexpr int LDSF0 = 2 * 6 * NP * 2 * 2 * 256 * 2;
  int grid;
  PROBE_RESET(ctx);
  KOCR_TRY((launch_persistent<conv_w43fh_kernel<NP, DIL>>(ctx, p, p.total_tiles, 256, LDSF0 + 4 * p.Cout_pad * 4, LDSF0 + W4_COEF_BYTES_MAX,
                                                           1, &grid)));
  {
    char what[64];
    snprintf(what, sizeof what, "conv_w43fh<%d> tiles %d steps %d", NP, p.total_tiles, p.nsteps);
    (void)what;
    PROBE_REPORT(ctx, what, grid);
  }
  return KOCR_OK;
}

int launch_w43fh(kocr_ctx* ctx, W4Params& p, int pieces) {
  if (p.dil != 1) return w4fh_launch<2, 1>(ctx, p);
  return pieces == 2 ? w4fh_launch<2>(ctx, p) : w4fh_launch<1>(ctx, p);
}
```

### keras_ocr_amd/csrc/w43_common.h

```cpp
#pragma once
#include "split_common.h"
#include <type_traits>
#include <cmath>
#include <algorithm>
#include <vector>

struct W4Params {
  const float* in;
  const unsigned short* wgt;
  float* out;
  const float* pre_a;
  const float* pre_b;
  const float* post_a;
  const float* post_b;
  int H, W, Cin, in_cs, in_co;
  int Cout, Cout_pad, out_cs, out_co;
  int relu;
  int nsteps;
  int Mtotal;
  int total_mtiles;
  float* pool_out;
  int pool_cs, pool_co, write_full, tiles_per_row;
  int total_tiles;
  int n_mpairs;
  int dil;
  int qpr;
  int m_fastest;
  unsigned* amax_out;
  unsigned* amax_pool;
  unsigned dv_tpr[2];
  unsigned dv_hh[2];
  unsigned dv_mp[2];
  unsigned dv_nb[2];
  unsigned dv_hw[2];
  const unsigned* amax_in;
  int Wv;
  unsigned dv_w[2];
  int rq_per_img;
  unsigned dv_rq[2];
  unsigned dv_qpr[2], dv_dil[2], dv_h[2];
  int cellW, cellWv, cells_per_row;
  unsigned dv_wc[2];
};

static inline void w4_div_magic(unsigned d, unsigned (&out)[2]) {
  if (d <= 1) {
    out[0] = 0;
    out[1] = 0;
    return;
  }
  unsigned L = 0;
  while ((1ull << L) < d) ++L;
  out[0] = (unsigned)(((1ull << 32) * ((1ull << L) - d)) / d + 1);
  out[1] = L - 1;
}

namespace {

__device__ __forceinline__ unsigned w4_fdiv(unsigned n, const unsigned (&dv)[2]) {
  if (dv[0] == 0 && dv[1] == 0) return n;
  const unsigned t = __umulhi(n, dv[0]);
  return (t + ((n - t) >> 1)) >> dv[1];
}

constexpr double W4_PA = 0.625, W4_PB = 1.5;
constexpr float W4_A = (float)W4_PA, W4_B = (float)W4_PB;
constexpr float W4_A2 = (float)(W4_PA * W4_PA), W4_B2 = (float)(W4_PB * W4_PB);
constexpr float W4_A3 = (float)(W4_PA * W4_PA * W4_PA), W4_B3 = (float)(W4_PB * W4_PB * W4_PB);
constexpr float W4_A2B2 = (float)(W4_PA * W4_PA * W4_PB * W4_PB), W4_A2PB2 = (float)(W4_PA * W4_PA + W4_PB * W4_PB);

constexpr int KH_STRIDE = 256;
constexpr int PLANE = 2 * 2 * KH_STRIDE;
constexpr int BUF = 6 * 3 * PLANE;
constexpr int LDS_BYTES = 2 * BUF * 2;

template <int POOL>
__device__ __forceinline__ long w4_mtile_pm0(const W4Params& p, int mt, int& y0, int& x0) {
  if constexpr (POOL) {
    const int rp_lin = (int)w4_fdiv((unsigned)mt, p.dv_tpr), cb = mt - rp_lin * p.tiles_per_row;
    const int hh = p.H >> 1;
    const int nimg = (int)w4_fdiv((unsigned)rp_lin, p.dv_hh), rp = rp_lin - nimg * hh;
    y0 = 2 * rp;
    x0 = cb * 64;
    return ((long)nimg * p.H + y0) * p.W + x0;
  } else {
    y0 = x0 = 0;
    return (long)mt * 128;
  }
}

__device__ __forceinline__ void w4_decode(const W4Params& p, int tile, int nblk_n, int& mp, int& nt) {
  const bool mf = p.m_fastest != 0;
  const unsigned dv[2] = {mf ? p.dv_mp[0] : p.dv_nb[0], mf ? p.dv_mp[1] : p.dv_nb[1]};
  const int quot = (int)w4_fdiv((unsigned)tile, dv);
  const int rem = tile - quot * (mf ? p.n_mpairs : nblk_n);
  nt = mf ? quot : rem;
  mp = mf ? rem : quot;
}

__device__ __forceinline__ void w4_stage_coef(const W4Params& p, float* coef, int tid) {
  for (int i = tid; i < p.Cout_pad; i += 256) {
    const int c = i < p.Cout ? i : p.Cout - 1;
    coef[i] = p.pre_a[c];
    coef[p.Cout_pad + i] = p.pre_b[c];
    coef[2 * p.Cout_pad + i] = p.post_a ? p.post_a[c] : 1.f;
    coef[3 * p.Cout_pad + i] = p.post_a ? p.post_b[c] : 0.f;
  }
}
constexpr int W4_COEF_BYTES_MAX = 4 * 1024 * 4;

__device__ __forceinline__ __amdgpu_buffer_rsrc_t w4_rsrc(const float* base, unsigned bytes) {
  const unsigned long long bb = (unsigned long long)base;
  const unsigned long long bbu = ((unsigned long long)(unsigned)__builtin_amdgcn_readfirstlane((int)(bb >> 32)) << 32) |
                                 (unsigned)__builtin_amdgcn_readfirstlane((int)bb);
  return __builtin_amdgcn_make_buffer_rsrc((void*)bbu, 0, (int)__builtin_amdgcn_readfirstlane((int)bytes), 0x00020000);
}

}

template <class T>
__device__ __forceinline__ T w4_transform(const T (&d)[6], int xi) {
  switch (xi) {
    case 0: return (W4_A2B2 * d[0] - W4_A2PB2 * d[2]) + d[4];
    case 1: return (d[4] - W4_B2 * d[2]) + W4_A * (d[3] - W4_B2 * d[1]);
    case 2: return (d[4] - W4_B2 * d[2]) - W4_A * (d[3] - W4_B2 * d[1]);
    case 3: return (d[4] - W4_A2 * d[2]) + W4_B * (d[3] - W4_A2 * d[1]);
    case 4: return (d[4] - W4_A2 * d[2]) - W4_B * (d[3] - W4_A2 * d[1]);
    default: return (W4_A2B2 * d[1] - W4_A2PB2 * d[3]) + d[5];
  }
}


__device__ __forceinline__ void w4_split_store(v4f V, unsigned short* pt, int slot, int plane) {
  u2v h, m, l;
  kocr_split4(V, h, m, l);
  unsigned short* dst = pt + slot;
  *reinterpret_cast<u2v*>(dst) = h;
  *reinterpret_cast<u2v*>(dst + plane) = m;
  *reinterpret_cast<u2v*>(dst + 2 * plane) = l;
}
__device__ __forceinline__ void w4_split_store(v2f V, unsigned short* pt, int slot, int plane) {
  unsigned h, m, l;
  kocr_split2(V, h, m, l);
  unsigned short* dst = pt + slot;
  *reinterpret_cast<unsigned*>(dst) = h;
  *reinterpret_cast<unsigned*>(dst + plane) = m;
  *reinterpret_cast<unsigned*>(dst + 2 * plane) = l;
}

__device__ __forceinline__ void w4_load_w(bf8 (&bw)[3], const unsigned short* w, int xi) {
#pragma unroll
  for (int s = 0; s < 3; ++s) bw[s] = *reinterpret_cast<const bf8*>(w + (size_t)(xi * 3 + s) * 64 * 8);
}

__device__ __forceinline__ void w4_mfma12(f16v (&acc)[2], const bf8 (&a)[2][3], const bf8 (&bw)[3]) {
  const bf8 b0 = bw[0], b1 = bw[1], b2 = bw[2];
#pragma unroll
  for (int m = 0; m < 2; ++m) acc[m] = __builtin_amdgcn_mfma_f32_32x32x16_bf16(a[m][2], b0, acc[m], 0, 0, 0);
#pragma unroll
  for (int m = 0; m < 2; ++m) acc[m] = __builtin_amdgcn_mfma_f32_32x32x16_bf16(a[m][0], b2, acc[m], 0, 0, 0);
#pragma unroll
  for (int m = 0; m < 2; ++m) acc[m] = __builtin_amdgcn_mfma_f32_32x32x16_bf16(a[m][1], b1, acc[m], 0, 0, 0);
#pragma unroll
  for (int m = 0; m < 2; ++m) acc[m] = __builtin_amdgcn_mfma_f32_32x32x16_bf16(a[m][1], b0, acc[m], 0, 0, 0);
#pragma unroll
  for (int m = 0; m < 2; ++m) acc[m] = __builtin_amdgcn_mfma_f32_32x32x16_bf16(a[m][0], b1, acc[m], 0, 0, 0);
#pragma unroll
  for (int m = 0; m < 2; ++m) acc[m] = __builtin_amdgcn_mfma_f32_32x32x16_bf16(a[m][0], b0, acc[m], 0, 0, 0);
}

__device__ __forceinline__ void w4_advance(int& ld_cg, bool& ld_next, int ncg) {
  const bool wrap = ld_cg == ncg - 1;
  ld_cg = wrap ? 0 : ld_cg + 1;
  ld_next = ld_next || wrap;
}


template <class Act>
__device__ __forceinline__ v4f w4_inverse(Act&& act, float m0, float m1, float m2, float m3, float m4, float m5) {
  const float s12 = m1 + m2, d12 = m1 - m2, s34 = m3 + m4, d34 = m3 - m4;
  return v4f{act((m0 + s12) + s34), act(W4_A * d12 + W4_B * d34), act(W4_A2 * s12 + W4_B2 * s34),
             act((W4_A3 * d12 + W4_B3 * d34) + m5)};
}

__device__ __forceinline__ int w4_opaque_stride(int cs) {
  int cs4 = cs * 4;
  asm volatile("" : "+s"(cs4));
  return cs4;
}
```

Before: 258.1.

## Re-read kernel params in epilogue and carry tile weight pointers across iterations

Adds a helper that reloads the kernel argument struct through an opaque kernarg pointer, so epilogue and geometry code read params fresh from scalar memory. The intent is to avoid keeping many param values live in SGPRs across the main loop. Tile decode for weight pointers now happens once in make_geo and is carried to the next iteration, instead of running two decodes per loop iteration. Accumulator zeroing is folded into the first step via a compile-time flag. The cost is extra scalar loads in the epilogue and more complex control flow.

```diff
diff --git a/keras_ocr_amd/csrc/conv_w43h.hip b/keras_ocr_amd/csrc/conv_w43h.hip
--- a/keras_ocr_amd/csrc/conv_w43h.hip
+++ b/keras_ocr_amd/csrc/conv_w43h.hip
@@ -42,7 +42,6 @@
   const int tid = threadIdx.x, lane = tid & 63;
   const int wn = __builtin_amdgcn_readfirstlane(tid >> 6);
   const int l31 = lane & 31, l5 = lane >> 5;
-  const int nblk_n = p.Cout_pad >> 7;
   const int total = p.total_tiles;
   const int ncg = p.Cin >> 4;
   const int ns = 3 * ncg;
@@ -56,7 +55,7 @@
     else
       return w * ROW_STRIDE + kh * KHS + ((q * 8) ^ (kh * 32));
   };
-  auto tile_org = [&](int mp, int& y0, int& x0, int& nimg_o) -> long {
+  auto tile_org = [&](const W4Params& p, int mp, int& y0, int& x0, int& nimg_o) -> long {
     if constexpr (MODE != 0) {
       const int rq = (int)w4_fdiv((unsigned)mp, p.dv_tpr), cb = mp - rq * p.tiles_per_row;
       const int nimg = (int)w4_fdiv((unsigned)rq, p.dv_rq), ro = rq - nimg * p.rq_per_img;
@@ -91,11 +90,12 @@
     int e1, qb;
     const float* base;
   };
-  auto make_geo = [&](int L, Geo& g, bool& left, bool& right) __attribute__((always_inline)) {
-    int mp, nt_unused;
-    w4_decode(p, kocr_xcd_remap(L < total ? L : 0, total), nblk_n, mp, nt_unused);
+  auto make_geo = [&](const W4Params& p, int L, Geo& g, bool& left, bool& right, int& nt) __attribute__((always_inline)) {
+    const int total = p.total_tiles;
+    int mp;
+    w4_decode(p, kocr_xcd_remap(L < total ? L : 0, total), p.Cout_pad >> 7, mp, nt);
     int y0, x0, nimg = 0;
-    const long pm = tile_org(mp, y0, x0, nimg);
+    const long pm = tile_org(p, mp, y0, x0, nimg);
     g.base = p.in + (pm * p.in_cs + p.in_co) - (long)(p.W + 1) * p.in_cs;
     const int tid = wn * 64 + kocr_fresh_lane();
     const int q4 = tid & 3, qd0 = (tid >> 2) & (QPR - 1), r0 = GEO == 2 ? (tid >> 5) : (tid >> 6);
@@ -343,23 +343,20 @@
   };
 
   w4_stage_coef(p, coef, tid);
-  make_geo(blockIdx.x, gc, lc, rc);
-  make_geo(blockIdx.x + G, gn, ln, rn);
+  int nt_c, nt_n;
+  make_geo(p, blockIdx.x, gc, lc, rc, nt_c);
+  make_geo(p, blockIdx.x + G, gn, ln, rn, nt_n);
   load_item0(raw0);
   load_item1(raw1);
   advance();
-  {
-    int mp0, nt0;
-    w4_decode(p, kocr_xcd_remap(blockIdx.x, total), nblk_n, mp0, nt0);
-    const unsigned w0 = w_tile(nt0);
-#pragma unroll
-    for (int st = 0; st < 2; ++st)
-#pragma unroll
-      for (int xi = 0; xi < 6; ++xi)
-#pragma unroll
-        for (int s = 0; s < NP; ++s)
-          bw[st][xi][s] = __builtin_bit_cast(hf8, __builtin_amdgcn_raw_buffer_load_b128(wrsrc, wlane, (int)(w0 + st * w_step + (unsigned)(xi * 2 + s) * 1024u), 0));
-  }
+  unsigned w_ptr = w_tile(nt_c), w_after = w_tile(nt_n);
+#pragma unroll
+  for (int st = 0; st < 2; ++st)
+#pragma unroll
+    for (int xi = 0; xi < 6; ++xi)
+#pragma unroll
+      for (int s = 0; s < NP; ++s)
+        bw[st][xi][s] = __builtin_bit_cast(hf8, __builtin_amdgcn_raw_buffer_load_b128(wrsrc, wlane, (int)(w_ptr + st * w_step + (unsigned)(xi * 2 + s) * 1024u), 0));
 #pragma unroll
   for (int xi = 0; xi < 6; ++xi) {
     produce4(raw0, As, xi, 0, kocr_pow2(gc.e), kocr_pow2(gc.e1), gc.qb);
@@ -373,10 +370,6 @@
 
   PROBE_RESTART();
   for (int L = blockIdx.x; L < total; L += G) {
-    int mp, nt, mp_n, nt_n;
-    w4_decode(p, kocr_xcd_remap(L, total), nblk_n, mp, nt);
-    w4_decode(p, kocr_xcd_remap(L + G < total ? L + G : L, total), nblk_n, mp_n, nt_n);
-    const unsigned w_ptr = w_tile(nt), w_after = w_tile(nt_n);
     auto w_at = [&](int s) { return s < ns ? w_ptr + (unsigned)s * w_step : w_after + (unsigned)(s - ns) * w_step; };
     const float s_cur = kocr_pow2(gc.e), s_nxt = kocr_pow2(gn.e);
     const float s_cur1 = kocr_pow2(gc.e1), s_nxt1 = kocr_pow2(gn.e1);
@@ -415,37 +408,41 @@
     }
     PROBE_T(0);
 
+    constexpr bool REREAD = POOL || GEO == 2 || MODE == 2;
+    const W4Params& pt = REREAD ? w4_params_again() : p;
     {
+      int mp, nt;
+      w4_decode(pt, kocr_xcd_remap(L, total), pt.Cout_pad >> 7, mp, nt);
       const int lane_e = kocr_fresh_lane();
       const int l31e = lane_e & 31, l5e = lane_e >> 5;
       const int n = (nt * 4 + wn) * 32 + l31e;
       int ty0, tx0, timg = 0;
-      const long tpm = tile_org(mp, ty0, tx0, timg);
+      const long tpm = tile_org(pt, mp, ty0, tx0, timg);
       int nimg, nimg1 = 0, cell0_x = 0;
       if constexpr (MODE == 2) {
-        const int j0 = (int)w4_fdiv((unsigned)tx0, p.dv_wc);
-        const int j1 = j0 + 1 < p.cells_per_row ? j0 + 1 : j0;
-        nimg = __builtin_amdgcn_readfirstlane(timg * p.cells_per_row + j0);
-        nimg1 = __builtin_amdgcn_readfirstlane(timg * p.cells_per_row + j1);
-        cell0_x = j0 * p.cellW;
+        const int j0 = (int)w4_fdiv((unsigned)tx0, pt.dv_wc);
+        const int j1 = j0 + 1 < pt.cells_per_row ? j0 + 1 : j0;
+        nimg = __builtin_amdgcn_readfirstlane(timg * pt.cells_per_row + j0);
+        nimg1 = __builtin_amdgcn_readfirstlane(timg * pt.cells_per_row + j1);
+        cell0_x = j0 * pt.cellW;
       } else if constexpr (MODE == 1) {
         nimg = __builtin_amdgcn_readfirstlane(timg);
       } else {
-        nimg = __builtin_amdgcn_readfirstlane((int)w4_fdiv((unsigned)tpm, p.dv_hw));
-      }
-      const unsigned seen_out = p.amax_out ? kocr_amax_peek(p.amax_out + nimg) : 0u;
-      const unsigned seen_pool = p.amax_pool ? kocr_amax_peek(p.amax_pool + nimg) : 0u;
+        nimg = __builtin_amdgcn_readfirstlane((int)w4_fdiv((unsigned)tpm, pt.dv_hw));
+      }
+      const unsigned seen_out = pt.amax_out ? kocr_amax_peek(pt.amax_out + nimg) : 0u;
+      const unsigned seen_pool = pt.amax_pool ? kocr_amax_peek(pt.amax_pool + nimg) : 0u;
       unsigned seen_out1 = 0u, seen_pool1 = 0u;
       if constexpr (MODE == 2) {
-        seen_out1 = p.amax_out ? kocr_amax_peek(p.amax_out + nimg1) : 0u;
-        seen_pool1 = p.amax_pool ? kocr_amax_peek(p.amax_pool + nimg1) : 0u;
-      }
-      const float pa = coef[n] * unscale, pb = coef[p.Cout_pad + n];
+        seen_out1 = pt.amax_out ? kocr_amax_peek(pt.amax_out + nimg1) : 0u;
+        seen_pool1 = pt.amax_pool ? kocr_amax_peek(pt.amax_pool + nimg1) : 0u;
+      }
+      const float pa = coef[n] * unscale, pb = coef[pt.Cout_pad + n];
       const float pa1 = coef[n] * unscale1;
-      const bool has_post = p.post_a != nullptr;
-      const float qa = coef[2 * p.Cout_pad + n], qb = coef[3 * p.Cout_pad + n];
-      const bool live = n < p.Cout;
-      const float lo = p.relu ? 0.f : -INFINITY;
+      const bool has_post = pt.post_a != nullptr;
+      const float qa = coef[2 * pt.Cout_pad + n], qb = coef[3 * pt.Cout_pad + n];
+      const bool live = n < pt.Cout;
+      const float lo = pt.relu ? 0.f : -INFINITY;
       auto act = [&](float v, float a) { return fmaxf(v * a + pb, lo); };
       const int l5q = 4 * l5e;
       auto qx_of = [&](int r) { return GEO == 2 ? (r & 3) + l5q : (r & 3) + 8 * ((r >> 2) & 1) + l5q; };
@@ -477,20 +474,20 @@
 #pragma unroll
         for (int r = 0; r < 16; ++r) {
           const int qx = qx_of(r);
-          const int cx = tx0 + 4 * qx - (qx < qb_cur ? cell0_x : cell0_x + p.cellW);
+          const int cx = tx0 + 4 * qx - (qx < qb_cur ? cell0_x : cell0_x + pt.cellW);
 #pragma unroll
           for (int j = 0; j < 4; ++j) {
-            const bool v = cx + j < p.cellWv;
+            const bool v = cx + j < pt.cellWv;
 #pragma unroll
             for (int m = 0; m < 2; ++m) acc[j][m][r] = (v && !(top && first_row(m, r))) ? acc[j][m][r] : 0.f;
           }
         }
       }
-      int ocs4 = p.out_cs * 4;
+      int ocs4 = pt.out_cs * 4;
       asm volatile("" : "+s"(ocs4));
-      int pcs4 = p.pool_cs * 4;
+      int pcs4 = pt.pool_cs * 4;
       asm volatile("" : "+s"(pcs4));
-      if (p.amax_out || p.amax_pool) {
+      if (pt.amax_out || pt.amax_pool) {
         if constexpr (MODE == 2) {
           float mx0 = 0.f, mx1 = 0.f;
 #pragma unroll
@@ -506,11 +503,11 @@
           }
           mx0 = live ? mx0 : 0.f;
           mx1 = live ? mx1 : 0.f;
-          if (p.amax_out) kocr_amax_update_known(p.amax_out + nimg, mx0, seen_out);
-          if (p.amax_pool) kocr_amax_update_known(p.amax_pool + nimg, mx0, seen_pool);
+          if (pt.amax_out) kocr_amax_update_known(pt.amax_out + nimg, mx0, seen_out);
+          if (pt.amax_pool) kocr_amax_update_known(pt.amax_pool + nimg, mx0, seen_pool);
           if (qb_cur < QPR) {
-            if (p.amax_out) kocr_amax_update_known(p.amax_out + nimg1, mx1, seen_out1);
-            if (p.amax_pool) kocr_amax_update_known(p.amax_pool + nimg1, mx1, seen_pool1);
+            if (pt.amax_out) kocr_amax_update_known(pt.amax_out + nimg1, mx1, seen_out1);
+            if (pt.amax_pool) kocr_amax_update_known(pt.amax_pool + nimg1, mx1, seen_pool1);
           }
         } else {
           float mx = 0.f;
@@ -521,21 +518,21 @@
 #pragma unroll
               for (int r = 0; r < 16; ++r) mx = fmaxf(mx, fabsf(acc[j][m][r]));
           mx = live ? mx : 0.f;
-          if (p.amax_out) kocr_amax_update_known(p.amax_out + nimg, mx, seen_out);
-          if (p.amax_pool) kocr_amax_update_known(p.amax_pool + nimg, mx, seen_pool);
+          if (pt.amax_out) kocr_amax_update_known(pt.amax_out + nimg, mx, seen_out);
+          if (pt.amax_pool) kocr_amax_update_known(pt.amax_pool + nimg, mx, seen_pool);
         }
       }
       PROBE_T(2);
       if constexpr (GEO == 2) {
-        const __amdgpu_buffer_rsrc_t ro = w4_rsrc(p.out + (tpm * p.out_cs + p.out_co), 0x7FFFFFFFu);
-        const unsigned vo = live ? (unsigned)((16 * l5e * p.out_cs + n) * 4) : OOB;
-        const int wlim = p.W - tx0 - 16 * l5e;
+        const __amdgpu_buffer_rsrc_t ro = w4_rsrc(pt.out + (tpm * pt.out_cs + pt.out_co), 0x7FFFFFFFu);
+        const unsigned vo = live ? (unsigned)((16 * l5e * pt.out_cs + n) * 4) : OOB;
+        const int wlim = pt.W - tx0 - 16 * l5e;
 #pragma unroll
         for (int m = 0; m < 2; ++m)
 #pragma unroll
           for (int r = 0; r < 16; ++r) {
-            const int px = (4 * m + (r >> 2)) * p.W + 4 * (r & 3);
-            if (MODE == 1 && ty0 + 4 * m + (r >> 2) >= p.H) continue;
+            const int px = (4 * m + (r >> 2)) * pt.W + 4 * (r & 3);
+            if (MODE == 1 && ty0 + 4 * m + (r >> 2) >= pt.H) continue;
 #pragma unroll
             for (int j = 0; j < 4; ++j) {
               const unsigned vom = MODE == 1 ? (4 * (r & 3) + j < wlim ? vo : OOB) : vo;
@@ -545,23 +542,23 @@
       } else {
 #pragma unroll
         for (int m = 0; m < 2; ++m) {
-          const long pm = tpm + (long)2 * m * p.W;
+          const long pm = tpm + (long)2 * m * pt.W;
           const int x0 = tx0;
-          if (!POOL || p.write_full) {
-            const __amdgpu_buffer_rsrc_t ro = w4_rsrc(p.out + (pm * p.out_cs + p.out_co), 0x7FFFFFFFu);
-            const unsigned vo = live ? (unsigned)((16 * l5e * p.out_cs + n) * 4) : OOB;
+          if (!POOL || pt.write_full) {
+            const __amdgpu_buffer_rsrc_t ro = w4_rsrc(pt.out + (pm * pt.out_cs + pt.out_co), 0x7FFFFFFFu);
+            const unsigned vo = live ? (unsigned)((16 * l5e * pt.out_cs + n) * 4) : OOB;
             if constexpr (MODE == 1) {
-              const int wlim = p.W - tx0 - 16 * l5e;
+              const int wlim = pt.W - tx0 - 16 * l5e;
 #pragma unroll
               for (int h = 0; h < 2; ++h) {
-                if (ty0 + 2 * m + h >= p.H) continue;
+                if (ty0 + 2 * m + h >= pt.H) continue;
 #pragma unroll
                 for (int r = 0; r < 8; ++r) {
                   const int px = 4 * ((r & 3) + 8 * (r >> 2));
 #pragma unroll
                   for (int j = 0; j < 4; ++j)
                     __builtin_amdgcn_raw_buffer_store_b32(__float_as_uint(acc[j][m][r + 8 * h]), ro, px + j < wlim ? vo : OOB,
-                                                          (px + j + h * p.W) * ocs4, 0);
+                                                          (px + j + h * pt.W) * ocs4, 0);
                 }
               }
             } else {
@@ -571,7 +568,7 @@
 #pragma unroll
                 for (int j = 0; j < 4; ++j) {
                   __builtin_amdgcn_raw_buffer_store_b32(__float_as_uint(acc[j][m][r]), ro, vo, (px + j) * ocs4, 0);
-                  __builtin_amdgcn_raw_buffer_store_b32(__float_as_uint(acc[j][m][r + 8]), ro, vo, (px + j + p.W) * ocs4, 0);
+                  __builtin_amdgcn_raw_buffer_store_b32(__float_as_uint(acc[j][m][r + 8]), ro, vo, (px + j + pt.W) * ocs4, 0);
                 }
               }
             }
@@ -579,13 +576,13 @@
           if constexpr (POOL) {
             long pp0;
             if constexpr (MODE == 1)
-              pp0 = ((long)timg * (p.H >> 1) + (ty0 >> 1) + m) * (p.W >> 1) + (x0 >> 1);
+              pp0 = ((long)timg * (pt.H >> 1) + (ty0 >> 1) + m) * (pt.W >> 1) + (x0 >> 1);
             else
               pp0 = ((pm - x0) >> 2) + (x0 >> 1);
-            const __amdgpu_buffer_rsrc_t rp = w4_rsrc(p.pool_out + (pp0 * p.pool_cs + p.pool_co), 0x7FFFFFFFu);
-            const unsigned vp = live ? (unsigned)((8 * l5e * p.pool_cs + n) * 4) : OOB;
-            if (MODE == 1 && (ty0 >> 1) + m >= (p.H >> 1)) continue;
-            const int plim = (p.W >> 1) - (x0 >> 1) - 8 * l5e;
+            const __amdgpu_buffer_rsrc_t rp = w4_rsrc(pt.pool_out + (pp0 * pt.pool_cs + pt.pool_co), 0x7FFFFFFFu);
+            const unsigned vp = live ? (unsigned)((8 * l5e * pt.pool_cs + n) * 4) : OOB;
+            if (MODE == 1 && (ty0 >> 1) + m >= (pt.H >> 1)) continue;
+            const int plim = (pt.W >> 1) - (x0 >> 1) - 8 * l5e;
             const bool ztop = MODE == 2 && ty0 == 0 && m == 0;
 #pragma unroll
             for (int r = 0; r < 8; ++r) {
@@ -607,7 +604,9 @@
     gc = gn;
     lc = ln;
     rc = rn;
-    make_geo(L + 2 * G, gn, ln, rn);
+    w_ptr = w_after;
+    make_geo(pt, L + 2 * G, gn, ln, rn, nt_n);
+    w_after = w_tile(nt_n);
     ld_next = false;
     PROBE_T(1);
   }
@@ -633,11 +632,11 @@
   const int G = gridDim.x;
   constexpr unsigned OOB = 0x80000000u;
 
-  auto tile_mt = [&](int mp, int m) {
+  auto tile_mt = [&](const W4Params& p, int mp, int m) {
     const int rq = (int)w4_fdiv((unsigned)mp, p.dv_tpr), cb = mp - rq * p.tiles_per_row;
     return (2 * rq + m) * p.tiles_per_row + cb;
   };
-  auto mtile_org = [&](int mp, int m, int& y0, int& x0, int& nimg_o) -> long {
+  auto mtile_org = [&](const W4Params& p, int mp, int m, int& y0, int& x0, int& nimg_o) -> long {
     if constexpr (MODE == 1) {
       const int rq = (int)w4_fdiv((unsigned)mp, p.dv_tpr), cb = mp - rq * p.tiles_per_row;
       const int nimg = (int)w4_fdiv((unsigned)rq, p.dv_rq), ro = rq - nimg * p.rq_per_img;
@@ -646,7 +645,7 @@
       nimg_o = nimg;
       return ((long)nimg * p.H + y0) * p.W + x0;
     } else {
-      const long pm = w4_mtile_pm0<1>(p, tile_mt(mp, m), y0, x0);
+      const long pm = w4_mtile_pm0<1>(p, tile_mt(p, mp, m), y0, x0);
       nimg_o = (int)w4_fdiv((unsigned)pm, p.dv_hw);
       return pm;
     }
@@ -663,10 +662,11 @@
     int e;
     const float* base;
   };
-  auto make_geo = [&](int L, Geo& g, bool& left, bool& right) __attribute__((always_inline)) {
+  auto make_geo = [&](const W4Params& p, int L, Geo& g, bool& left, bool& right) __attribute__((always_inline)) {
+    const int total = p.total_tiles;
     const int mp = kocr_xcd_remap(L < total ? L : 0, total);
     int y0, x0, nimg;
-    const long pm = mtile_org(mp, 0, y0, x0, nimg);
+    const long pm = mtile_org(p, mp, 0, y0, x0, nimg);
     g.base = p.in + (pm * p.in_cs + p.in_co) - (long)(p.W + 1) * p.in_cs;
     const int tid = wave * 64 + kocr_fresh_lane();
     const int q4 = tid & 3, qd0 = (tid >> 2) & (QPR - 1), r0 = tid >> 6;
@@ -849,8 +849,8 @@
   };
 
   w4_stage_coef(p, coef, tid);
-  make_geo(blockIdx.x, gc, lc, rc);
-  make_geo(blockIdx.x + G, gn, ln, rn);
+  make_geo(p, blockIdx.x, gc, lc, rc);
+  make_geo(p, blockIdx.x + G, gn, ln, rn);
   load_item0(raw0[0]);
   load_item1(raw1[0]);
   advance();
@@ -890,20 +890,21 @@
     }
 
     PROBE_T(0);
+    const W4Params& pt = w4_params_again();
     {
       const int lane_e = kocr_fresh_lane();
       const int l31e = lane_e & 31, l5e = lane_e >> 5;
       const int n = wn * 32 + l31e;
       int y0, x0, timg;
-      const long pm = mtile_org(mp, ph, y0, x0, timg);
+      const long pm = mtile_org(pt, mp, ph, y0, x0, timg);
       const int nimg = __builtin_amdgcn_readfirstlane(timg);
-      const unsigned seen_out = p.amax_out ? kocr_amax_peek(p.amax_out + nimg) : 0u;
-      const unsigned seen_pool = p.amax_pool ? kocr_amax_peek(p.amax_pool + nimg) : 0u;
-      const float pa = coef[n] * unscale, pb = coef[p.Cout_pad + n];
-      const bool has_post = p.post_a != nullptr;
-      const float qa = coef[2 * p.Cout_pad + n], qb = coef[3 * p.Cout_pad + n];
-      const bool live = n < p.Cout;
-      const float lo = p.relu ? 0.f : -INFINITY;
+      const unsigned seen_out = pt.amax_out ? kocr_amax_peek(pt.amax_out + nimg) : 0u;
+      const unsigned seen_pool = pt.amax_pool ? kocr_amax_peek(pt.amax_pool + nimg) : 0u;
+      const float pa = coef[n] * unscale, pb = coef[pt.Cout_pad + n];
+      const bool has_post = pt.post_a != nullptr;
+      const float qa = coef[2 * pt.Cout_pad + n], qb = coef[3 * pt.Cout_pad + n];
+      const bool live = n < pt.Cout;
+      const float lo = pt.relu ? 0.f : -INFINITY;
       auto act = [&](float v) { return fmaxf(v * pa + pb, lo); };
       v4f* xch = reinterpret_cast<v4f*>(As + BUF_R);
       float out[4][16];
@@ -986,35 +987,35 @@
           for (int j = 0; j < 4; ++j) out[j][r] = out[j][r] * qa + qb;
       }
       if constexpr (OCC == 1) __syncthreads();
-      int ocs4 = p.out_cs * 4;
+      int ocs4 = pt.out_cs * 4;
       asm volatile("" : "+s"(ocs4));
-      int pcs4 = p.pool_cs * 4;
+      int pcs4 = pt.pool_cs * 4;
       asm volatile("" : "+s"(pcs4));
-      if (p.amax_out || p.amax_pool) {
+      if (pt.amax_out || pt.amax_pool) {
         float mx = 0.f;
 #pragma unroll
         for (int j = 0; j < 4; ++j)
 #pragma unroll
           for (int r = 0; r < 16; ++r) mx = fmaxf(mx, fabsf(out[j][r]));
         mx = live ? mx : 0.f;
-        if (p.amax_out) kocr_amax_update_known(p.amax_out + nimg, mx, seen_out);
-        if (p.amax_pool) kocr_amax_update_known(p.amax_pool + nimg, mx, seen_pool);
+        if (pt.amax_out) kocr_amax_update_known(pt.amax_out + nimg, mx, seen_out);
+        if (pt.amax_pool) kocr_amax_update_known(pt.amax_pool + nimg, mx, seen_pool);
       }
       PROBE_T(2);
-      if (!POOL || p.write_full) {
-        const __amdgpu_buffer_rsrc_t ro = w4_rsrc(p.out + (pm * p.out_cs + p.out_co), 0x7FFFFFFFu);
-        const unsigned vo = live ? (unsigned)((16 * l5e * p.out_cs + n) * 4) : OOB;
+      if (!POOL || pt.write_full) {
+        const __amdgpu_buffer_rsrc_t ro = w4_rsrc(pt.out + (pm * pt.out_cs + pt.out_co), 0x7FFFFFFFu);
+        const unsigned vo = live ? (unsigned)((16 * l5e * pt.out_cs + n) * 4) : OOB;
         if constexpr (MODE == 1) {
-          const int wlim = p.W - x0 - 16 * l5e;
+          const int wlim = pt.W - x0 - 16 * l5e;
 #pragma unroll
           for (int h = 0; h < 2; ++h) {
-            if (y0 + h >= p.H) continue;
+            if (y0 + h >= pt.H) continue;
 #pragma unroll
             for (int r = 0; r < 8; ++r) {
               const int px = 4 * ((r & 3) + 8 * (r >> 2));
 #pragma unroll
               for (int j = 0; j < 4; ++j)
-                __builtin_amdgcn_raw_buffer_store_b32(__float_as_uint(out[j][r + 8 * h]), ro, px + j < wlim ? vo : OOB, (px + j + h * p.W) * ocs4, 0);
+                __builtin_amdgcn_raw_buffer_store_b32(__float_as_uint(out[j][r + 8 * h]), ro, px + j < wlim ? vo : OOB, (px + j + h * pt.W) * ocs4, 0);
             }
           }
         } else {
@@ -1024,7 +1025,7 @@
 #pragma unroll
             for (int j = 0; j < 4; ++j) {
               __builtin_amdgcn_raw_buffer_store_b32(__float_as_uint(out[j][r]), ro, vo, (px + j) * ocs4, 0);
-              __builtin_amdgcn_raw_buffer_store_b32(__float_as_uint(out[j][r + 8]), ro, vo, (px + j + p.W) * ocs4, 0);
+              __builtin_amdgcn_raw_buffer_store_b32(__float_as_uint(out[j][r + 8]), ro, vo, (px + j + pt.W) * ocs4, 0);
             }
           }
         }
@@ -1032,13 +1033,13 @@
       if constexpr (POOL) {
         long pp0;
         if constexpr (MODE == 1)
-          pp0 = ((long)timg * (p.H >> 1) + (y0 >> 1)) * (p.W >> 1) + (x0 >> 1);
+          pp0 = ((long)timg * (pt.H >> 1) + (y0 >> 1)) * (pt.W >> 1) + (x0 >> 1);
         else
           pp0 = ((pm - x0) >> 2) + (x0 >> 1);
-        const __amdgpu_buffer_rsrc_t rp = w4_rsrc(p.pool_out + (pp0 * p.pool_cs + p.pool_co), 0x7FFFFFFFu);
-        const unsigned vp = live ? (unsigned)((8 * l5e * p.pool_cs + n) * 4) : OOB;
-        const bool prow = MODE != 1 || (y0 >> 1) < (p.H >> 1);
-        const int plim = (p.W >> 1) - (x0 >> 1) - 8 * l5e;
+        const __amdgpu_buffer_rsrc_t rp = w4_rsrc(pt.pool_out + (pp0 * pt.pool_cs + pt.pool_co), 0x7FFFFFFFu);
+        const unsigned vp = live ? (unsigned)((8 * l5e * pt.pool_cs + n) * 4) : OOB;
+        const bool prow = MODE != 1 || (y0 >> 1) < (pt.H >> 1);
+        const int plim = (pt.W >> 1) - (x0 >> 1) - 8 * l5e;
         if (prow) {
 #pragma unroll
           for (int r = 0; r < 8; ++r) {
@@ -1055,7 +1056,7 @@
     gc = gn;
     lc = ln;
     rc = rn;
-    make_geo(L + 2 * G, gn, ln, rn);
+    make_geo(pt, L + 2 * G, gn, ln, rn);
     ld_next = false;
     PROBE_T(1);
   }
@@ -1072,11 +1073,9 @@
   const int tid = threadIdx.x, lane = tid & 63;
   const int wn = __builtin_amdgcn_readfirstlane(tid >> 6);
   const int l31 = lane & 31, l5 = lane >> 5;
-  const int nblk_n = p.Cout_pad >> 7;
   const int total = p.total_tiles;
   const int ns = p.nsteps;
   const int G = gridDim.x;
-  const int hw = p.H * p.W;
   constexpr unsigned OOB = 0x80000000u;
 
   const int qi = tid >> 2, q4 = tid & 3;
@@ -1090,9 +1089,11 @@
     const float* base;
   };
   const int dd = DIL ? p.dil : 1;
-  auto make_geo = [&](int L, Geo& g) __attribute__((always_inline)) {
-    int mp, nt_unused;
-    w4_decode(p, kocr_xcd_remap(L < total ? L : 0, total), nblk_n, mp, nt_unused);
+  auto make_geo = [&](const W4Params& p, int L, Geo& g, int& nt) __attribute__((always_inline)) {
+    const int total = p.total_tiles, hw = p.H * p.W;
+    const int dd = DIL ? p.dil : 1;
+    int mp;
+    w4_decode(p, kocr_xcd_remap(L < total ? L : 0, total), p.Cout_pad >> 7, mp, nt);
     const int tid_f = wn * 64 + kocr_fresh_lane();
     const int qi = tid_f >> 2, q4 = tid_f & 3;
     if constexpr (DIL) {
@@ -1190,18 +1191,21 @@
 #pragma unroll
       for (int m = 0; m < 2; ++m) a[m][s] = *reinterpret_cast<const hf8*>(base + s * PLANE_F + m * 2 * KH_STRIDE);
   };
-  auto mfma_pt = [&](const hf8 (&a)[2][NP], int xi) __attribute__((always_inline)) {
+  auto mfma_pt = [&](auto first_c, const hf8 (&a)[2][NP], int xi) __attribute__((always_inline)) {
+    constexpr bool FIRST = decltype(first_c)::value;
+    const f16v zero = {};
     if constexpr (NP == 2) {
 #pragma unroll
-      for (int m = 0; m < 2; ++m) acc[xi][m] = __builtin_amdgcn_mfma_f32_32x32x16_f16(a[m][1], bw[xi][0], acc[xi][m], 0, 0, 0);
+      for (int m = 0; m < 2; ++m) acc[xi][m] = __builtin_amdgcn_mfma_f32_32x32x16_f16(a[m][1], bw[xi][0], FIRST ? zero : acc[xi][m], 0, 0, 0);
 #pragma unroll
       for (int m = 0; m < 2; ++m) acc[xi][m] = __builtin_amdgcn_mfma_f32_32x32x16_f16(a[m][0], bw[xi][1], acc[xi][m], 0, 0, 0);
     }
 #pragma unroll
-    for (int m = 0; m < 2; ++m) acc[xi][m] = __builtin_amdgcn_mfma_f32_32x32x16_f16(a[m][0], bw[xi][0], acc[xi][m], 0, 0, 0);
+    for (int m = 0; m < 2; ++m)
+      acc[xi][m] = __builtin_amdgcn_mfma_f32_32x32x16_f16(a[m][0], bw[xi][0], (FIRST && NP == 1) ? zero : acc[xi][m], 0, 0, 0);
   };
   hf8 a0[2][NP], a1[2][NP];
-  auto step = [&](const unsigned short* bufc, unsigned short* bufn, const v4f (&raw)[6], const unsigned short* w_next, float sk)
+  auto step = [&](auto first_c, const unsigned short* bufc, unsigned short* bufn, const v4f (&raw)[6], const unsigned short* w_next, float sk)
                   __attribute__((always_inline)) {
     auto load_b = [&](int xi) __attribute__((always_inline)) {
 #pragma unroll
@@ -1223,7 +1227,7 @@
       __builtin_amdgcn_sched_barrier(0);
       load_a(a1, bufc, 2 * q + 1);
       produce_point(raw, bufn, 2 * q, sk);
-      mfma_pt(a0, 2 * q);
+      mfma_pt(first_c, a0, 2 * q);
       interleave();
       __builtin_amdgcn_sched_barrier(0);
       load_b(2 * q);
@@ -1231,14 +1235,14 @@
       if (q < 2) {
         load_a(a0, bufc, 2 * q + 2);
         produce_point(raw, bufn, 2 * q + 1, sk);
-        mfma_pt(a1, 2 * q + 1);
+        mfma_pt(first_c, a1, 2 * q + 1);
         interleave();
       } else {
         produce_point(raw, bufn, 5, sk);
         __syncthreads();
         load_a(a0, bufn, 0);
         __builtin_amdgcn_sched_barrier(0);
-        mfma_pt(a1, 5);
+        mfma_pt(first_c, a1, 5);
       }
       __builtin_amdgcn_sched_barrier(0);
       load_b(2 * q + 1);
@@ -1246,20 +1250,17 @@
   };
 
   w4_stage_coef(p, coef, tid);
-  make_geo(blockIdx.x, gc);
-  make_geo(blockIdx.x + G, gn);
+  int nt_c, nt_n;
+  make_geo(p, blockIdx.x, gc, nt_c);
+  make_geo(p, blockIdx.x + G, gn, nt_n);
+  const unsigned short *w_ptr = w_tile(nt_c), *w_after = w_tile(nt_n);
   v4f rawA[6], rawB[6];
   load_raw(rawA);
   load_raw(rawB);
-  {
-    int mp0, nt0;
-    w4_decode(p, kocr_xcd_remap(blockIdx.x, total), nblk_n, mp0, nt0);
-    const unsigned short* w0 = w_tile(nt0);
-#pragma unroll
-    for (int xi = 0; xi < 6; ++xi)
-#pragma unroll
-      for (int s = 0; s < NP; ++s) bw[xi][s] = *reinterpret_cast<const hf8*>(w0 + (size_t)(xi * 2 + s) * 64 * 8);
-  }
+#pragma unroll
+  for (int xi = 0; xi < 6; ++xi)
+#pragma unroll
+    for (int s = 0; s < NP; ++s) bw[xi][s] = *reinterpret_cast<const hf8*>(w_ptr + (size_t)(xi * 2 + s) * 64 * 8);
 #pragma unroll
   for (int xi = 0; xi < 6; ++xi) produce_point(rawA, As, xi, gc.s);
   load_raw(rawA);
@@ -1268,50 +1269,45 @@
 
   PROBE_T0();
   for (int L = blockIdx.x; L < total; L += G) {
-    int mp, nt, mp_n, nt_n;
-    w4_decode(p, kocr_xcd_remap(L, total), nblk_n, mp, nt);
-    w4_decode(p, kocr_xcd_remap(L + G < total ? L + G : L, total), nblk_n, mp_n, nt_n);
-    const unsigned short* w_ptr = w_tile(nt);
-    const unsigned short* w_after = w_tile(nt_n);
     const float s_cur = gc.s, s_nxt = gn.s;
-#pragma unroll
-    for (int x = 0; x < 6; ++x)
-#pragma unroll
-      for (int m = 0; m < 2; ++m)
-#pragma unroll
-        for (int r = 0; r < 16; ++r) acc[x][m][r] = 0.f;
     __builtin_amdgcn_s_waitcnt(0x0F70);
-    for (int s = 0; s < ns; s += 2) {
-      step(As, As + BUF_F, rawB, w_ptr + (size_t)(s + 1) * w_step, s_cur);
+    auto pair = [&](auto first_c, int s) __attribute__((always_inline)) {
+      step(first_c, As, As + BUF_F, rawB, w_ptr + (size_t)(s + 1) * w_step, s_cur);
       load_raw(rawB);
-      step(As + BUF_F, As, rawA, s + 2 < ns ? w_ptr + (size_t)(s + 2) * w_step : w_after, s + 2 < ns ? s_cur : s_nxt);
+      step(std::false_type{}, As + BUF_F, As, rawA, s + 2 < ns ? w_ptr + (size_t)(s + 2) * w_step : w_after, s + 2 < ns ? s_cur : s_nxt);
       load_raw(rawA);
-    }
+    };
+    pair(std::true_type{}, 0);
+    for (int s = 2; s < ns; s += 2) pair(std::false_type{}, s);
     PROBE_T(0);
     const int e0c = gc.e0, e1c = gc.e1;
 
+    const W4Params& pt = w4_params_again();
     {
+      int mp, nt;
+      w4_decode(pt, kocr_xcd_remap(L, total), pt.Cout_pad >> 7, mp, nt);
+      const int hw = pt.H * pt.W, dd = DIL ? pt.dil : 1;
       const int lane_e = kocr_fresh_lane();
       const int l31e = lane_e & 31, l5e = lane_e >> 5;
       const int n = (nt * 4 + wn) * 32 + l31e;
       const long pm0 = (long)mp * 256;
-      const long pm0c = pm0 < (long)p.Mtotal ? pm0 : (long)p.Mtotal - 1;
-      const int n0 = __builtin_amdgcn_readfirstlane((int)w4_fdiv((unsigned)pm0c, p.dv_hw));
+      const long pm0c = pm0 < (long)pt.Mtotal ? pm0 : (long)pt.Mtotal - 1;
+      const int n0 = __builtin_amdgcn_readfirstlane((int)w4_fdiv((unsigned)pm0c, pt.dv_hw));
       const long b1 = ((long)(n0 + 1) * hw - pm0) >> 2;
       const int qb = __builtin_amdgcn_readfirstlane((int)(b1 < 64 ? b1 : 64));
-      const int n1 = ((long)(n0 + 1) * hw < (long)p.Mtotal) ? n0 + 1 : n0;
+      const int n1 = ((long)(n0 + 1) * hw < (long)pt.Mtotal) ? n0 + 1 : n0;
       unsigned seen0 = 0, seen1 = 0;
-      if (p.amax_out) {
-        seen0 = kocr_amax_peek(p.amax_out + n0);
-        seen1 = kocr_amax_peek(p.amax_out + n1);
+      if (pt.amax_out) {
+        seen0 = kocr_amax_peek(pt.amax_out + n0);
+        seen1 = kocr_amax_peek(pt.amax_out + n1);
       }
       const float u0 = kocr_pow2(-e0c), u1 = kocr_pow2(-e1c);
-      const float pre_a = coef[n], pb = coef[p.Cout_pad + n];
+      const float pre_a = coef[n], pb = coef[pt.Cout_pad + n];
       const float pa0 = pre_a * u0, pa1 = pre_a * u1;
-      const bool has_post = p.post_a != nullptr;
-      const bool live = n < p.Cout;
-      const float lo = p.relu ? 0.f : -INFINITY;
-      const int qlim = (int)((((long)p.Mtotal - pm0) >> 2) < 64 ? (((long)p.Mtotal - pm0) >> 2) : 64);
+      const bool has_post = pt.post_a != nullptr;
+      const bool live = n < pt.Cout;
+      const float lo = pt.relu ? 0.f : -INFINITY;
+      const int qlim = (int)((((long)pt.Mtotal - pm0) >> 2) < 64 ? (((long)pt.Mtotal - pm0) >> 2) : 64);
       const int l5q = 4 * l5e;
 #pragma unroll
       for (int m = 0; m < 2; ++m)
@@ -1328,7 +1324,7 @@
           acc[3][m][r] = fmaxf(((W4_A3 * d12 + W4_B3 * d34) + m5) * pa + pb, lo);
         }
       if (has_post) {
-        const float qa = coef[2 * p.Cout_pad + n], qb_ = coef[3 * p.Cout_pad + n];
+        const float qa = coef[2 * pt.Cout_pad + n], qb_ = coef[3 * pt.Cout_pad + n];
 #pragma unroll
         for (int j = 0; j < 4; ++j)
 #pragma unroll
@@ -1336,19 +1332,19 @@
 #pragma unroll
             for (int r = 0; r < 16; ++r) acc[j][m][r] = acc[j][m][r] * qa + qb_;
       }
-      if (!DIL && p.Wv) {
+      if (!DIL && pt.Wv) {
 #pragma unroll
         for (int m = 0; m < 2; ++m)
 #pragma unroll
           for (int r = 0; r < 16; ++r) {
             const int q = m * 32 + (r & 3) + 8 * (r >> 2) + l5q;
             const unsigned pq = (unsigned)(pm0 + 4 * q);
-            const int x0 = (int)(pq - w4_fdiv(pq, p.dv_w) * (unsigned)p.W);
-#pragma unroll
-            for (int j = 0; j < 4; ++j) acc[j][m][r] = x0 + j < p.Wv ? acc[j][m][r] : 0.f;
+            const int x0 = (int)(pq - w4_fdiv(pq, pt.dv_w) * (unsigned)pt.W);
+#pragma unroll
+            for (int j = 0; j < 4; ++j) acc[j][m][r] = x0 + j < pt.Wv ? acc[j][m][r] : 0.f;
           }
       }
-      if (p.amax_out) {
+      if (pt.amax_out) {
         float mx0 = 0.f, mx1 = 0.f;
 #pragma unroll
         for (int m = 0; m < 2; ++m)
@@ -1359,16 +1355,16 @@
             mx0 = fmaxf(mx0, q < qb ? mq : 0.f);
             mx1 = fmaxf(mx1, q < qb ? 0.f : mq);
           }
-        kocr_amax_update_known(p.amax_out + n0, mx0, seen0);
-        if (qb < 64) kocr_amax_update_known(p.amax_out + n1, mx1, seen1);
+        kocr_amax_update_known(pt.amax_out + n0, mx0, seen0);
+        if (qb < 64) kocr_amax_update_known(pt.amax_out + n1, mx1, seen1);
       }
       PROBE_T(2);
-      int ocs4 = p.out_cs * 4;
+      int ocs4 = pt.out_cs * 4;
       asm volatile("" : "+s"(ocs4));
       if constexpr (DIL) {
         const unsigned q0 = (unsigned)mp * 64u;
-        const unsigned row_a = w4_fdiv(q0, p.dv_qpr);
-        const __amdgpu_buffer_rsrc_t ro = w4_rsrc(p.out + ((long)row_a * p.W * p.out_cs + p.out_co), 0x7FFFFFFFu);
+        const unsigned row_a = w4_fdiv(q0, pt.dv_qpr);
+        const __amdgpu_buffer_rsrc_t ro = w4_rsrc(pt.out + ((long)row_a * pt.W * pt.out_cs + pt.out_co), 0x7FFFFFFFu);
         const int dstep = dd * ocs4;
 #pragma unroll
         for (int m = 0; m < 2; ++m)
@@ -1376,19 +1372,19 @@
           for (int r = 0; r < 16; ++r) {
             const int q = m * 32 + (r & 3) + 8 * (r >> 2) + l5q;
             const unsigned qg = q0 + (unsigned)q;
-            const unsigned row = w4_fdiv(qg, p.dv_qpr);
-            const int qr = (int)(qg - row * (unsigned)p.qpr);
-            const int qd = (int)w4_fdiv((unsigned)qr, p.dv_dil);
+            const unsigned row = w4_fdiv(qg, pt.dv_qpr);
+            const int qr = (int)(qg - row * (unsigned)pt.qpr);
+            const int qd = (int)w4_fdiv((unsigned)qr, pt.dv_dil);
             const int x0 = qd * 4 * dd + (qr - qd * dd);
-            const unsigned vo = (live && q < qlim) ? (unsigned)((((int)(row - row_a) * p.W + x0) * p.out_cs + n) * 4) : OOB;
+            const unsigned vo = (live && q < qlim) ? (unsigned)((((int)(row - row_a) * pt.W + x0) * pt.out_cs + n) * 4) : OOB;
 #pragma unroll
             for (int j = 0; j < 4; ++j) __builtin_amdgcn_raw_buffer_store_b32(__float_as_uint(acc[j][m][r]), ro, vo, j * dstep, 0);
           }
       } else {
-      const long rem = ((long)p.Mtotal - pm0) * ocs4;
+      const long rem = ((long)pt.Mtotal - pm0) * ocs4;
       const __amdgpu_buffer_rsrc_t ro =
-          w4_rsrc(p.out + (pm0 * p.out_cs + p.out_co), rem < 0x7FFFFFFFL ? (unsigned)(rem > 0 ? rem : 0) : 0x7FFFFFFFu);
-      const unsigned vo = live ? (unsigned)((16 * l5e * p.out_cs + n) * 4) : OOB;
+          w4_rsrc(pt.out + (pm0 * pt.out_cs + pt.out_co), rem < 0x7FFFFFFFL ? (unsigned)(rem > 0 ? rem : 0) : 0x7FFFFFFFu);
+      const unsigned vo = live ? (unsigned)((16 * l5e * pt.out_cs + n) * 4) : OOB;
 #pragma unroll
       for (int m = 0; m < 2; ++m)
 #pragma unroll
@@ -1402,7 +1398,9 @@
       PROBE_T(3);
     }
     gc = gn;
-    make_geo(L + 2 * G, gn);
+    w_ptr = w_after;
+    make_geo(pt, L + 2 * G, gn, nt_n);
+    w_after = w_tile(nt_n);
     ld_next = false;
     PROBE_T(1);
   }
diff --git a/keras_ocr_amd/csrc/w43_common.h b/keras_ocr_amd/csrc/w43_common.h
--- a/keras_ocr_amd/csrc/w43_common.h
+++ b/keras_ocr_amd/csrc/w43_common.h
@@ -116,6 +116,12 @@
   return __builtin_amdgcn_make_buffer_rsrc((void*)bbu, 0, (int)__builtin_amdgcn_readfirstlane((int)bytes), 0x00020000);
 }
 
+__device__ __forceinline__ const W4Params& w4_params_again() {
+  auto q = (const __attribute__((address_space(4))) W4Params*)__builtin_amdgcn_kernarg_segment_ptr();
+  asm volatile("" : "+s"(q));
+  return *(const W4Params*)q;
+}
+
 }
 
 template <class T>
```

Result: no change. 260.1, median of 6 (+0.7%).
